# openxrlab/xrsfm

Hardware: AMD Instinct MI355X
Metric: BA iterations/sec x (cams+points) (higher is better)
Workload: dtype f64; 1 GPU; synthetic BAL-style L: 1000 cams / 500000 points / 2000000 obs, GBA accurate (ba_solver.cc:626-629), seed 4; parallelism=single GPU, linear_solver=cholesky (explicit reduced camera matrix, exact)

## Files before the change

xrsfm_amd/csrc/ba_chol.h:

```cpp
#pragma once
#include "ba_kernels.h"
#include "ba_pack.h"

namespace xba {

constexpr int kNB = 64;
constexpr int kLdT = 66;
constexpr int kCamsPerTileDev = 10;

struct CholDev {
    int n, n_pad, T;
    double* S;
    const int* tmap; size_t ld; size_t tstride;
    double* Linv;
    double* y;
    double* rhs;
    double* x;
    const int* cam_off;
    const int* tile_rows;
    int cw, cpt;
};

__device__ __forceinline__ double* tile_ptr(const CholDev& c, int i, int k) {
    return c.tmap ? c.S + (size_t)c.tmap[i * c.T + k] * c.tstride : c.S + (size_t)(i * kNB) * c.ld + k * kNB;
}

typedef double v4d __attribute__((ext_vector_type(4)));

constexpr int kRedLd = 15;

constexpr int kGramTabLd = kGramMaxCams + 1;
static_assert(kTileRunLd == kGramMaxCams, "one run record per distinct camera of a Gram tile (ba_kernels.h: k_gram_runs)");

template <bool UPPER>
__device__ __forceinline__ void pairs_V(const double* F, const double* E, const double* __restrict__ hc, double* V) {
#pragma unroll
    for (int a = 0; a < 6; ++a) {
        const double w0 = F[a] * E[0] + F[6 + a] * E[3], w1 = F[a] * E[1] + F[6 + a] * E[4], w2 = F[a] * E[2] + F[6 + a] * E[5];
        if (UPPER) {
            V[3 * a + 0] = w0 * hc[0];
            V[3 * a + 1] = w0 * hc[1] + w1 * hc[3];
            V[3 * a + 2] = w0 * hc[2] + w1 * hc[4] + w2 * hc[5];
        } else {
            V[3 * a + 0] = w0 * hc[0] + w1 * hc[1] + w2 * hc[2];
            V[3 * a + 1] = w1 * hc[3] + w2 * hc[4];
            V[3 * a + 2] = w2 * hc[5];
        }
    }
}

template <bool UPPER>
__device__ __forceinline__ void pairs_diag(const double* F, const double* V, const double* __restrict__ hc,
                                           const double* __restrict__ g, double* o28) {
    int idx = 0;
#pragma unroll
    for (int a = 0; a < 6; ++a)
#pragma unroll
        for (int c2 = a; c2 < 6; ++c2)
            o28[idx++] = F[a] * F[c2] + F[6 + a] * F[6 + c2]
                         - (V[3 * a] * V[3 * c2] + V[3 * a + 1] * V[3 * c2 + 1] + V[3 * a + 2] * V[3 * c2 + 2]);
    const double g0 = g[0], g1 = g[1], g2 = g[2];
    const double u0 = UPPER ? hc[0] * g0 : hc[0] * g0 + hc[1] * g1 + hc[2] * g2;
    const double u1 = UPPER ? hc[1] * g0 + hc[3] * g1 : hc[3] * g1 + hc[4] * g2;
    const double u2 = UPPER ? hc[2] * g0 + hc[4] * g1 + hc[5] * g2 : hc[5] * g2;
#pragma unroll
    for (int a = 0; a < 6; ++a) o28[21 + a] = -(V[3 * a] * u0 + V[3 * a + 1] * u1 + V[3 * a + 2] * u2);
    o28[27] = 0.0;
}

struct SGroup { int idx, len; double* base; int wld; double ds0, ds1; int dofs; };
template <int NV, typename V>
__device__ __forceinline__ bool sgroup_finish(SGroup g, V (&v)[NV], double* __restrict__ scat, int lane) {
    constexpr int W = sizeof(V) / sizeof(double);
    if (g.idx > 0) {
#pragma unroll
        for (int i = 0; i < NV * W; ++i) g.base[i * kWave + lane] = reinterpret_cast<const double*>(&v[i / W])[i % W];
        g.base[NV * W * kWave + lane] = g.ds0;
        g.base[(NV * W + 1) * kWave + lane] = g.ds1;
    }
    __syncthreads();
    if (g.idx > 0) return false;
    for (int j = 1; j < g.len; ++j) {
        const double* src = g.base + (size_t)j * g.wld;
#pragma unroll
        for (int i = 0; i < NV; ++i) {
            if constexpr (W == 1) v[i] += src[i * kWave + lane];
            else {
#pragma unroll
                for (int q = 0; q < W; ++q) v[i][q] += src[(i * W + q) * kWave + lane];
            }
        }
        g.ds0 += src[NV * W * kWave + lane];
        g.ds1 += src[(NV * W + 1) * kWave + lane];
    }
    if (g.dofs >= 0) { scat[g.dofs] = g.ds0; scat[g.dofs + 14] = g.ds1; }
    return true;
}

template <int NI, int CW = 6>
__device__ __forceinline__ void gram_tile(double* __restrict__ Vst, int R, int Cp, int C, const int* __restrict__ dtab,
                                          double* __restrict__ scat2, int lane, const double (&V)[3 * CW], bool valid, int t, int cidx,
                                          int T, int Th, int passes, bool dense, SGroup sg = SGroup{0, 1, nullptr, 0, 0.0, 0.0, -1},
                                          double* __restrict__ scat = nullptr) {
    static_assert(NI >= 1 && NI <= 4, "a Gram tile has at most 10 cameras = 60 operand rows (ba_pack.h: kGramMaxCams)");
    const int li = lane & 15, lk = lane >> 4;
    v4d acc[NI * (NI + 1) / 2];
#pragma unroll
    for (int p = 0; p < NI * (NI + 1) / 2; ++p) acc[p] = (v4d){0.0, 0.0, 0.0, 0.0};
    const double* rowp[NI];
#pragma unroll
    for (int I = 0; I < NI; ++I) rowp[I] = Vst + min(16 * I + li, R - 1) * Cp + lk;
    for (int h = 0; h < passes; ++h) {
        const int t0 = h * Th, tn = min(Th, T - t0);
        const int C4 = (3 * tn + 3) & ~3;
        if (dense && passes == 1) {
            const int padc = C4 - 3 * tn;
            for (int e = lane; e < R * padc; e += kWave) {
                const int row = e / padc, cc = 3 * tn + (e - row * padc);
                Vst[row * Cp + cc] = 0.0;
            }
        } else {
            for (int e = lane; e < (R * Cp) / 2; e += kWave) reinterpret_cast<double2*>(Vst)[e] = make_double2(0.0, 0.0);
            if (((R * Cp) & 1) && lane == kWave - 1) Vst[R * Cp - 1] = 0.0;
        }
        if (valid && t >= t0 && t < t0 + tn) {
#pragma unroll
            for (int i = 0; i < CW; ++i)
#pragma unroll
                for (int m = 0; m < 3; ++m) Vst[(CW * cidx + i) * Cp + 3 * (t - t0) + m] = V[3 * i + m];
        }
        __builtin_amdgcn_s_waitcnt(0xc07f);
        __builtin_amdgcn_wave_barrier();
        XBA_STAMP(0, 6);
        for (int k0 = 0; k0 < C4; k0 += 4) {
            double a[NI];
#pragma unroll
            for (int I = 0; I < NI; ++I) a[I] = rowp[I][k0];
            int p = 0;
#pragma unroll
            for (int I = 0; I < NI; ++I)
#pragma unroll
                for (int J = 0; J <= I; ++J) { acc[p] = __builtin_amdgcn_mfma_f64_16x16x4f64(a[I], a[J], acc[p], 0, 0, 0); ++p; }
        }
        __builtin_amdgcn_s_waitcnt(0xc07f);
        __builtin_amdgcn_wave_barrier();
    }
    XBA_STAMP(0, 7);
    if (NI <= 2 && sg.len > 1 && !sgroup_finish(sg, acc, scat, lane)) return;
    (void)C; (void)R;
    int tcol[NI], jcol[NI];
#pragma unroll
    for (int J = 0; J < NI; ++J) { const int col = 16 * J + li; const int ra = col / CW; tcol[J] = ra * kGramTabLd; jcol[J] = col - CW * ra; }
    int p = 0;
#pragma unroll
    for (int I = 0; I < NI; ++I) {
// ... 343 lines not shown
                    __builtin_amdgcn_wave_barrier();
                }
            } else if (cp >= 0) {
                double2* out = reinterpret_cast<double2*>(d.scat + 28 * (size_t)cp);
#pragma unroll
                for (int k = 0; k < 14; ++k) out[k] = make_double2(o28[2 * k], o28[2 * k + 1]);
            }
        }
        XBA_STAMP(0, 5);
        const int C = d.tile_ncam[it.first_tile];
        if (GRAM) {
            const unsigned long long headmask = __ballot(s.head);
            const int T = __popcll(headmask);
            const int nvalid = __popcll(__ballot(s.valid));
            const int t = __popcll(headmask & ((2ull << lane) - 1ull)) - 1;
            const int cidx = s.valid ? cidx_raw : 0;
            int passes = 1;
            (void)gram_lds_need(C, T, &passes);
            const int Th = (T + passes - 1) / passes;
            const int R = 6 * C, Rp = (R + 15) & ~15, Cp = ((3 * Th + 3) & ~3) + kGramPad;
            double* Vst = smem;
            int* dtab = reinterpret_cast<int*>(smem + R * Cp);
            dtab[lane] = dt0;
            if (lane + kWave < kGramTabLd * kGramTabLd) dtab[lane + kWave] = dt1;
            const bool dense = nvalid == T * C;
            (void)Rp;
            unsigned short* sched = reinterpret_cast<unsigned short*>(dtab + kGramTabLd * kGramTabLd);
            if (NIK <= 2 && g4_n > 0 && passes == 1) {
                gram4_sched_store(sched, g4_se, lane, g4_n);
                gram_tile4<6>(Vst, R, Cp, C, dtab, scat2, lane, V, s.valid, t, cidx, T, dense, sched, g4_n, sg, d.scat);
            }
            else if (NIK == 0) {
                if (R > 32) gram_tile<3>(Vst, R, Cp, C, dtab, scat2, lane, V, s.valid, t, cidx, T, Th, passes, dense, sg, d.scat);
                else if (R > 16) gram_tile<2>(Vst, R, Cp, C, dtab, scat2, lane, V, s.valid, t, cidx, T, Th, passes, dense, sg, d.scat);
                else gram_tile<1>(Vst, R, Cp, C, dtab, scat2, lane, V, s.valid, t, cidx, T, Th, passes, dense, sg, d.scat);
            }
            else gram_tile<(NIK > 0 ? NIK : 1)>(Vst, R, Cp, C, dtab, scat2, lane, V, s.valid, t, cidx, T, Th, passes, dense, sg, d.scat);
            XBA_STAMP(0, 8);
            return;
        }
        if (GRAM) return;
        if (pair_v) {
            if (s.valid) {
                double2* out = reinterpret_cast<double2*>(pair_v + 18 * (size_t)s.slot);
#pragma unroll
                for (int k = 0; k < 9; ++k) out[k] = make_double2(V[2 * k], V[2 * k + 1]);
            }
            return;
        }
        if (s.valid) {
            pbase = slot_pair_ptr[s.slot];
            npair = slot_pair_ptr[s.slot + 1] - pbase;
        }
        int maxp = npair;
#pragma unroll
        for (int off = 32; off > 0; off >>= 1) maxp = max(maxp, __shfl_xor(maxp, off, kWave));
        for (int dd = 1; dd <= maxp; ++dd) {
            double Vb[18];
#pragma unroll
            for (int k = 0; k < 18; ++k) Vb[k] = __shfl_down(V[k], dd, kWave);
            if (dd <= npair) {
                double2* out = reinterpret_cast<double2*>(scat2 + 36 * (size_t)pair_dst[pbase + dd - 1]);
#pragma unroll
                for (int rb = 0; rb < 6; ++rb) {
                    double o[6];
#pragma unroll
                    for (int ca = 0; ca < 6; ++ca)
                        o[ca] = Vb[3 * rb] * V[3 * ca] + Vb[3 * rb + 1] * V[3 * ca + 1] + Vb[3 * rb + 2] * V[3 * ca + 2];
                    out[3 * rb + 0] = make_double2(o[0], o[1]);
                    out[3 * rb + 1] = make_double2(o[2], o[3]);
                    out[3 * rb + 2] = make_double2(o[4], o[5]);
                }
            }
        }
        return;
    }
    if (GRAM) return;
    const int s_begin = it.first_tile * kWave, s_end = s_begin + it.n_tiles * kWave;
    for (int sa = s_begin + lane; sa < s_end; sa += kWave) {
        if (d.slot_cam[sa] < 0) continue;
        const int pt = d.slot_pt[sa];
        double hc[6];
        {
            const double* hp = (PREP ? d.Hpp : d.Hc) + 6 * (size_t)pt;
            double hv[6];
            for (int k = 0; k < 6; ++k) hv[k] = hp[k];
            if (PREP) point_factor(hv, radius, hc);
            else for (int k = 0; k < 6; ++k) hc[k] = hv[k];
        }
        double Va[18];
        {
            double Fa[12], Ea[6], o28[28], r0, r1;
            load_FE_rc(d, sa, d.slot_cam[sa], pt, Fa, Ea, r0, r1);
            pairs_V<PREP>(Fa, Ea, hc, Va);
            pairs_diag<PREP>(Fa, Va, hc, d.gp + 3 * (size_t)pt, o28);
            double* out = d.scat + 28 * (size_t)d.slot_campos_s[sa];
            for (int k = 0; k < 28; ++k) out[k] = o28[k];
        }
        if (pair_v) {
            double2* out = reinterpret_cast<double2*>(pair_v + 18 * (size_t)sa);
            for (int k = 0; k < 9; ++k) out[k] = make_double2(Va[2 * k], Va[2 * k + 1]);
            continue;
        }
        const int pbase = slot_pair_ptr[sa];
        const int npair = slot_pair_ptr[sa + 1] - pbase;
        for (int dd = 1; dd <= npair; ++dd) {
            const int sb = sa + dd;
            double Fb[12], Eb[6], Vb[18], r0, r1;
            load_FE_rc(d, sb, d.slot_cam[sb], pt, Fb, Eb, r0, r1);
            pairs_V<PREP>(Fb, Eb, hc, Vb);
            double* out = scat2 + 36 * (size_t)pair_dst[pbase + dd - 1];
            for (int rb = 0; rb < 6; ++rb)
                for (int ca = 0; ca < 6; ++ca)
                    out[6 * rb + ca] = Vb[3 * rb] * Va[3 * ca] + Vb[3 * rb + 1] * Va[3 * ca + 1] + Vb[3 * rb + 2] * Va[3 * ca + 2];
        }
    }
}

struct FillLists { const int* tiles; const int* tptr; const int* tent; const double* Sblk; const int* blk_rc;
                   double radius; };
template <int LD>
__device__ __forceinline__ void compose_tile(const CholDev& c, const Dev& d, const FillLists& f, int q, double* A, double* rl) {
    const int ti = f.tiles[2 * q], tj = f.tiles[2 * q + 1];
    const int t = threadIdx.x;
    const int nrows = c.tile_rows[ti];
    for (int e = t; e < kNB * kNB; e += 256) {
        const int r = e >> 6, col = e & 63;
        A[r * LD + col] = (ti == tj && r == col && r >= nrows) ? 1.0 : 0.0;
    }
    if (rl && t < kNB) rl[t] = 0.0;
    __syncthreads();
    const int q0 = f.tptr[q], q1 = f.tptr[q + 1];
    for (int w = t; w < (q1 - q0) * 36; w += 256) {
        const int ent = f.tent[q0 + w / 36], e = w % 36, r = e / 6, col = e % 6;
        if (ent >= 0) {
            const int orow = c.cam_off[f.blk_rc[2 * ent]], ocol = c.cam_off[f.blk_rc[2 * ent + 1]];
            const double v = -f.Sblk[36 * (size_t)ent + e];
            if (orow > ocol) A[((orow & 63) + r) * LD + (ocol & 63) + col] = v;
            else A[((ocol & 63) + col) * LD + (orow & 63) + r] = v;
        } else {
            const int cam = -ent - 1, o = c.cam_off[cam] & 63;
            const double* S = d.camS + 28 * (size_t)cam;
            if (col >= r) {
                double v = S[6 * r - r * (r - 1) / 2 + (col - r)];
                if (r == col) v += f.radius > 0.0 ? clampd(d.camlin[12 * (size_t)cam + r], kLmDiagMin, kLmDiagMax) / f.radius : d.Dc2[6 * (size_t)cam + r];
                A[(o + col) * LD + o + r] = v;
            }
            if (rl && e < 6) rl[o + e] = d.camlin[12 * (size_t)cam + 6 + e] + S[21 + e];
        }
    }
    __syncthreads();
}

__global__ __launch_bounds__(256) void k_tile_fill(CholDev c, Dev d, const int* __restrict__ tiles, const int* __restrict__ tptr,
                                                   const int* __restrict__ tent, const double* __restrict__ Sblk,
                                                   const int* __restrict__ blk_rc, double radius, const int* __restrict__ list = nullptr) {
    __shared__ double A[kNB * (kNB + 1)];
    __shared__ double rl[kNB];
    const FillLists f{tiles, tptr, tent, Sblk, blk_rc, radius};
    const int q = list ? list[blockIdx.x] : (int)blockIdx.x;
    const int ti = tiles[2 * q], tj = tiles[2 * q + 1];
    const int t = threadIdx.x;
    compose_tile<kNB + 1>(c, d, f, q, A, rl);
    double* base = tile_ptr(c, ti, tj);
    for (int e = t; e < kNB * kNB; e += 256) {
        const int r = e >> 6, col = e & 63;
        base[(size_t)r * c.ld + col] = A[r * (kNB + 1) + col];
    }
    if (ti == tj && t < kNB) c.rhs[ti * kNB + t] = rl[t];
}

__global__ void k_sol_gather(CholDev c, double* __restrict__ out, int n_cams) {
    const int i = blockIdx.x * blockDim.x + threadIdx.x;
    if (i < n_cams * c.cw) out[i] = c.x[c.cam_off[i / c.cw] + i % c.cw];
}

__device__ __forceinline__ double readlane_d(double v, int lane) {
    int lo = __double2loint(v), hi = __double2hiint(v);
    lo = __builtin_amdgcn_readlane(lo, lane);
    hi = __builtin_amdgcn_readlane(hi, lane);
    return __hiloint2double(hi, lo);
}
template <int L>
__device__ __forceinline__ double row_bcast_c(double v) {
    int lo = __double2loint(v), hi = __double2hiint(v);
    lo = __builtin_amdgcn_mov_dpp(lo, 0x150 + L, 0xf, 0xf, true);
    hi = __builtin_amdgcn_mov_dpp(hi, 0x150 + L, 0xf, 0xf, true);
    return __hiloint2double(hi, lo);
}
__device__ __forceinline__ double row_bcast(double v, int l) {
    switch (l) {
        case 0: return row_bcast_c<0>(v); case 1: return row_bcast_c<1>(v); case 2: return row_bcast_c<2>(v); case 3: return row_bcast_c<3>(v);
        case 4: return row_bcast_c<4>(v); case 5: return row_bcast_c<5>(v); case 6: return row_bcast_c<6>(v); case 7: return row_bcast_c<7>(v);
        case 8: return row_bcast_c<8>(v); case 9: return row_bcast_c<9>(v); case 10: return row_bcast_c<10>(v); case 11: return row_bcast_c<11>(v);
        case 12: return row_bcast_c<12>(v); case 13: return row_bcast_c<13>(v); case 14: return row_bcast_c<14>(v); default: return row_bcast_c<15>(v);
    }
}
template <int L>
__device__ __forceinline__ double row_bcast64_c(double v) {
    const long long x = __builtin_bit_cast(long long, v);
    const long long r = __builtin_amdgcn_update_dpp((long long)0, x, 0x150 + L, 0xf, 0xf, true);
    return __builtin_bit_cast(double, r);
}
__device__ __forceinline__ double row_bcast64(double v, int l) {
    switch (l) {
        case 0: return row_bcast64_c<0>(v); case 1: return row_bcast64_c<1>(v); case 2: return row_bcast64_c<2>(v); case 3: return row_bcast64_c<3>(v);
        case 4: return row_bcast64_c<4>(v); case 5: return row_bcast64_c<5>(v); case 6: return row_bcast64_c<6>(v); case 7: return row_bcast64_c<7>(v);
        case 8: return row_bcast64_c<8>(v); case 9: return row_bcast64_c<9>(v); case 10: return row_bcast64_c<10>(v); case 11: return row_bcast64_c<11>(v);
        case 12: return row_bcast64_c<12>(v); case 13: return row_bcast64_c<13>(v); case 14: return row_bcast64_c<14>(v); default: return row_bcast64_c<15>(v);
    }
}
#ifndef XBA_POTRF_PV
#define XBA_POTRF_PV 4
#endif
#ifndef XBA_POTRF_OVL
#define XBA_POTRF_OVL 1
#endif
__device__ __forceinline__ void allgather4(double v, double (&out)[4]) {
    const unsigned lo = (unsigned)__double2loint(v), hi = (unsigned)__double2hiint(v);
    const auto l1 = __builtin_amdgcn_permlane16_swap(lo, lo, false, false);
    const auto h1 = __builtin_amdgcn_permlane16_swap(hi, hi, false, false);
    const auto le = __builtin_amdgcn_permlane32_swap(l1[0], l1[0], false, false);
    const auto he = __builtin_amdgcn_permlane32_swap(h1[0], h1[0], false, false);
    const auto lo2 = __builtin_amdgcn_permlane32_swap(l1[1], l1[1], false, false);
    const auto ho2 = __builtin_amdgcn_permlane32_swap(h1[1], h1[1], false, false);
    out[0] = __hiloint2double((int)he[0], (int)le[0]); out[2] = __hiloint2double((int)he[1], (int)le[1]);
    out[1] = __hiloint2double((int)ho2[0], (int)lo2[0]); out[3] = __hiloint2double((int)ho2[1], (int)lo2[1]);
}
struct Panel4 { double a0, a1, a2, a3, x0, x1, x2, x3; };
template <int JJ>
__device__ __forceinline__ void potrf_panel_step(double& ak, double& xk, double& r, double& piv,
                                                 double* a_next, double* x_next, const int n_next) {
    piv = row_bcast64_c<JJ>(ak);
    r = fast_rcp(piv);
    const double tl = ak * r;
    const double xs = xk * r;
    if (n_next >= 1) { const double bv = row_bcast64_c<(JJ + 1) & 15>(ak); a_next[0] = fma(-tl, bv, a_next[0]); x_next[0] = fma(-bv, xs, x_next[0]); }
    if (n_next >= 2) { const double bv = row_bcast64_c<(JJ + 2) & 15>(ak); a_next[1] = fma(-tl, bv, a_next[1]); x_next[1] = fma(-bv, xs, x_next[1]); }
    if (n_next >= 3) { const double bv = row_bcast64_c<(JJ + 3) & 15>(ak); a_next[2] = fma(-tl, bv, a_next[2]); x_next[2] = fma(-bv, xs, x_next[2]); }
}
template <int P>
__device__ __forceinline__ void potrf_panel4(v4d& aa, v4d& ax, bool m1, bool m2, double& Lc, double& Xc, double& Pv) {
    double pa[4], px[4];
    allgather4(aa[P], pa);
    allgather4(ax[P], px);
    double a0 = pa[0], a1 = pa[1], a2 = pa[2], a3 = pa[3], x0 = px[0], x1 = px[1], x2 = px[2], x3 = px[3];
    double r0, r1, r2, r3, j0, j1, j2, j3;
    {
        double an[3] = {a1, a2, a3}, xn[3] = {x1, x2, x3};
        potrf_panel_step<4 * P + 0>(a0, x0, r0, j0, an, xn, 3);
        a1 = an[0]; a2 = an[1]; a3 = an[2]; x1 = xn[0]; x2 = xn[1]; x3 = xn[2];
    }
    {
        double an[3] = {a2, a3, 0.0}, xn[3] = {x2, x3, 0.0};
        potrf_panel_step<4 * P + 1>(a1, x1, r1, j1, an, xn, 2);
        a2 = an[0]; a3 = an[1]; x2 = xn[0]; x3 = xn[1];
    }
    {
        double an[3] = {a3, 0.0, 0.0}, xn[3] = {x3, 0.0, 0.0};
        potrf_panel_step<4 * P + 2>(a2, x2, r2, j2, an, xn, 1);
        a3 = an[0]; x3 = xn[0];
    }
    {
        double an[3] = {0.0, 0.0, 0.0}, xn[3] = {0.0, 0.0, 0.0};
        potrf_panel_step<4 * P + 3>(a3, x3, r3, j3, an, xn, 0);
    }
    auto sel = [&](double v0, double v1, double v2, double v3) { return m2 ? (m1 ? v3 : v2) : (m1 ? v1 : v0); };
    const double a_op = sel(a0, a1, a2, a3), x_op = sel(x0, x1, x2, x3), r_op = sel(r0, r1, r2, r3);
    if (P < 3) {
        const double na = -a_op;
        aa = __builtin_amdgcn_mfma_f64_16x16x4f64(na, a_op * r_op, aa, 0, 0, 0);
        ax = __builtin_amdgcn_mfma_f64_16x16x4f64(na, x_op * r_op, ax, 0, 0, 0);
    }
    Lc = a_op;
    Xc = x_op;
    Pv = sel(j0, j1, j2, j3);
}
__device__ __forceinline__ void potrf_block16_mfma(double (*A)[kLdT], double (*Li)[kLdT], int b0, int lane) {
    const int li = lane & 15, lk = lane >> 4;
    v4d aa, ax;
#pragma unroll
    for (int g = 0; g < 4; ++g) { aa[g] = A[b0 + li][b0 + lk + 4 * g]; ax[g] = (lk + 4 * g == li) ? 1.0 : 0.0; }
    const bool m1 = (lk & 1) != 0, m2 = (lk & 2) != 0;
    double L0, L1, L2, L3, X0, X1, X2, X3, u0, u1, u2, u3;
    potrf_panel4<0>(aa, ax, m1, m2, L0, X0, u0);
    potrf_panel4<1>(aa, ax, m1, m2, L1, X1, u1);
    potrf_panel4<2>(aa, ax, m1, m2, L2, X2, u2);
    potrf_panel4<3>(aa, ax, m1, m2, L3, X3, u3);
    {
        double y0 = __builtin_amdgcn_rsq(u0), y1 = __builtin_amdgcn_rsq(u1), y2 = __builtin_amdgcn_rsq(u2), y3 = __builtin_amdgcn_rsq(u3);
        const double h0 = 0.5 * u0, h1 = 0.5 * u1, h2 = 0.5 * u2, h3 = 0.5 * u3;
#pragma unroll
        for (int it = 0; it < 2; ++it) {
            const double f0 = fma(-h0 * y0, y0, 1.5), f1 = fma(-h1 * y1, y1, 1.5), f2 = fma(-h2 * y2, y2, 1.5), f3 = fma(-h3 * y3, y3, 1.5);
            y0 = y0 * f0; y1 = y1 * f1; y2 = y2 * f2; y3 = y3 * f3;
        }
        L0 *= y0; X0 *= y0; L1 *= y1; X1 *= y1; L2 *= y2; X2 *= y2; L3 *= y3; X3 *= y3;
    }
    A[b0 + li][b0 + lk] = (lk <= li) ? L0 : 0.0;             Li[b0 + lk][b0 + li] = X0;
    A[b0 + li][b0 + 4 + lk] = (4 + lk <= li) ? L1 : 0.0;     Li[b0 + 4 + lk][b0 + li] = X1;
    A[b0 + li][b0 + 8 + lk] = (8 + lk <= li) ? L2 : 0.0;     Li[b0 + 8 + lk][b0 + li] = X2;
    A[b0 + li][b0 + 12 + lk] = (12 + lk <= li) ? L3 : 0.0;   Li[b0 + 12 + lk][b0 + li] = X3;
}

template <int PV>
__device__ __forceinline__ void potrf_block16(double (*A)[kLdT], double (*Li)[kLdT], int b0, int lane) {
    if constexpr (PV == 4) { potrf_block16_mfma(A, Li, b0, lane); return; }
    const int li = lane & 15;
    double a[16];
#pragma unroll
    for (int cc = 0; cc < 16; ++cc) a[cc] = A[b0 + li][b0 + cc];
    double lcol[16];
#pragma unroll
    for (int r = 0; r < 16; ++r) lcol[r] = (r == li) ? 1.0 : 0.0;
#define XBA_POTRF_UPD(cc)                                                \
    {                                                                    \
        const double bv_ = (PV == 1) ? row_bcast64(a[jj], (cc)) : row_bcast(a[jj], (cc));        \
        a[(cc)] = fma(-tl, bv_, a[(cc)]);                                \
        lcol[(cc)] = fma(-bv_, xs, lcol[(cc)]);                          \
        asm volatile("" : "+v"(lcol[(cc)]));    \
    }
    double piv[16];
// ... 439 lines not shown
                                                        double* __restrict__ Wp) {
    __shared__ __attribute__((aligned(16))) double Rs[2][2][kNB * kLdQ];
    __shared__ __attribute__((aligned(16))) double Cs[2][2][kNB * kLdQ];
    __shared__ double yv[2][kNB];
    const int t = threadIdx.x, lane = t & 63, wave = t >> 6, wa = wave >> 1, wb = wave & 1;
    const int o = t >> 2, part = t & 3, li = lane & 15, lk = lane >> 4;
  {
    const int* e = mc + 8 * wg[blockIdx.x];
    const int i0 = e[0], i1 = e[1], k0 = e[2], k1 = e[3], q0 = e[4], q1 = e[5], out0 = e[6], stride = e[7];
    const int ia = wa ? i1 : i0, kb = wb ? k1 : k0;
    const bool active = ia >= 0 && ia >= kb;
    const bool diag = (i0 == k0);
    v4d acc[4][4];
#pragma unroll
    for (int m = 0; m < 4; ++m)
#pragma unroll
        for (int n2 = 0; n2 < 4; ++n2) acc[m][n2] = (v4d){0.0, 0.0, 0.0, 0.0};
    const int i1r = i1 >= 0 ? i1 : i0;
    auto load_step = [&](int st, v2d (&g0)[2], v2d (&g1)[2], v2d (&g2)[2], v2d (&g3)[2]) {
        const int j = q0 + (st >> 2), col = (st & 3) * 16;
        load_quarter_regs(g0, tile_ptr(c, i0, j) + col, c.ld); load_quarter_regs(g1, tile_ptr(c, i1r, j) + col, c.ld);
        load_quarter_regs(g2, tile_ptr(c, k0, j) + col, c.ld); load_quarter_regs(g3, tile_ptr(c, k1, j) + col, c.ld);
    };
    const int ns = 4 * (q1 - q0);
    v2d rg0[2], rg1[2], rg2[2], rg3[2];
    double yreg = 0.0;
    {
        load_step(0, rg0, rg1, rg2, rg3);
        if (diag && t < kNB) yreg = c.y[q0 * kNB + t];
        store_quarter_lds(Rs[0][0], rg0); store_quarter_lds(Rs[0][1], rg1);
        store_quarter_lds(Cs[0][0], rg2); store_quarter_lds(Cs[0][1], rg3);
        if (diag && t < kNB) yv[0][t] = yreg;
        if (ns > 1) {
            load_step(1, rg0, rg1, rg2, rg3);
        }
        __syncthreads();
    }
    double sv0 = 0.0, sv1 = 0.0;
    for (int s = 0; s < ns; ++s) {
        const int buf = s & 1;
        if (s + 1 < ns) {
            store_quarter_lds(Rs[buf ^ 1][0], rg0); store_quarter_lds(Rs[buf ^ 1][1], rg1);
            store_quarter_lds(Cs[buf ^ 1][0], rg2); store_quarter_lds(Cs[buf ^ 1][1], rg3);
            if (diag && ((s + 1) & 3) == 0 && t < kNB) yv[((s + 1) >> 2) & 1][t] = yreg;
        }
        if (s + 2 < ns) {
            load_step(s + 2, rg0, rg1, rg2, rg3);
            if (diag && ((s + 2) & 3) == 0 && t < kNB) yreg = c.y[(q0 + ((s + 2) >> 2)) * kNB + t];
        }
        if (diag) {
            const double* yq = yv[(s >> 2) & 1] + (s & 3) * 16 + part * 4;
#pragma unroll
            for (int m = 0; m < 4; ++m) {
                sv0 += Rs[buf][0][o * kLdQ + part * 4 + m] * yq[m];
                sv1 += Rs[buf][1][o * kLdQ + part * 4 + m] * yq[m];
            }
        }
        if (active) {
            const double* As = Rs[buf][wa];
            const double* Bs = Cs[buf][wb];
#pragma unroll
            for (int kk = 0; kk < 16; kk += 4) {
                double a[4], b[4];
#pragma unroll
                for (int m = 0; m < 4; ++m) {
                    a[m] = As[(16 * m + li) * kLdQ + kk + lk];
                    b[m] = Bs[(16 * m + li) * kLdQ + kk + lk];
                }
#pragma unroll
                for (int m = 0; m < 4; ++m)
#pragma unroll
                    for (int n2 = 0; n2 < 4; ++n2) acc[m][n2] = __builtin_amdgcn_mfma_f64_16x16x4f64(a[m], b[n2], acc[m][n2], 0, 0, 0);
            }
        }
        __syncthreads();
    }
    if (active) {
        double* out = Wp + (size_t)(out0 + (2 * wa + wb) * stride) * kPartStride;
#pragma unroll
        for (int m = 0; m < 4; ++m)
#pragma unroll
            for (int n2 = 0; n2 < 4; ++n2)
#pragma unroll
                for (int g = 0; g < 4; ++g) out[(16 * m + lk + 4 * g) * kNB + 16 * n2 + li] = acc[m][n2][g];
    }
    if (diag) {
        sv0 += __shfl_xor(sv0, 1, kWave); sv0 += __shfl_xor(sv0, 2, kWave);
        sv1 += __shfl_xor(sv1, 1, kWave); sv1 += __shfl_xor(sv1, 2, kWave);
        if (part == 0) {
            Wp[(size_t)out0 * kPartStride + kNB * kNB + o] = sv0;
            if (i1 >= 0) Wp[(size_t)(out0 + 3 * stride) * kPartStride + kNB * kNB + o] = sv1;
        }
    }
  }
}

__device__ __forceinline__ double sum_strided(const double* __restrict__ base, size_t stride, int n) {
    double s = 0.0;
    int p = 0;
    for (; p + 8 <= n; p += 8) {
        double v[8];
#pragma unroll
        for (int u = 0; u < 8; ++u) v[u] = base[(size_t)(p + u) * stride];
        s += ((v[0] + v[1]) + (v[2] + v[3])) + ((v[4] + v[5]) + (v[6] + v[7]));
    }
    for (; p < n; ++p) s += base[(size_t)p * stride];
    return s;
}

template <int EPT>
__device__ __forceinline__ void ll_update_reduce_body(const CholDev& c, const int bx, const int by, const int* __restrict__ rt,
                                                      const int* __restrict__ rp, const double* __restrict__ Wp) {
    const int i = rt[2 * bx], k = rt[2 * bx + 1];
    const int p0 = rp[2 * bx], p1 = rp[2 * bx + 1];
    if (EPT == 1) {
        const int e = by * 256 + threadIdx.x;
        const double s = sum_strided(Wp + (size_t)p0 * kPartStride + e, kPartStride, p1 - p0);
        tile_ptr(c, i, k)[(size_t)(e >> 6) * c.ld + (e & 63)] -= s;
    } else {
        double s[EPT], a0[EPT];
        const double* W = Wp + (size_t)p0 * kPartStride + (size_t)by * EPT * 256 + threadIdx.x;
        double* const tik = tile_ptr(c, i, k);
#pragma unroll
        for (int u = 0; u < EPT; ++u) { s[u] = 0.0; a0[u] = tik[(size_t)(((by * EPT + u) * 256 + threadIdx.x) >> 6) * c.ld + (threadIdx.x & 63)]; }
        int p = p0;
        for (; p + 2 <= p1; p += 2) {
            double v0[EPT], v1[EPT];
#pragma unroll
            for (int u = 0; u < EPT; ++u) { v0[u] = W[(size_t)u * 256]; v1[u] = W[kPartStride + (size_t)u * 256]; }
#pragma unroll
            for (int u = 0; u < EPT; ++u) { s[u] += v0[u]; s[u] += v1[u]; }
            W += 2 * kPartStride;
        }
        if (p < p1) {
#pragma unroll
            for (int u = 0; u < EPT; ++u) s[u] += W[(size_t)u * 256];
        }
#pragma unroll
        for (int u = 0; u < EPT; ++u) {
            const int e = (by * EPT + u) * 256 + threadIdx.x;
            tik[(size_t)(e >> 6) * c.ld + (e & 63)] = a0[u] - s[u];
        }
    }
    if (i == k && by == 0 && threadIdx.x < kNB) {
        const double s = sum_strided(Wp + (size_t)p0 * kPartStride + kNB * kNB + threadIdx.x, kPartStride, p1 - p0);
        c.rhs[k * kNB + threadIdx.x] -= s;
    }
}
__global__ __launch_bounds__(256) void k_ll_update_reduce(CholDev c, const int* __restrict__ rt, const int* __restrict__ rp,
                                                          const double* __restrict__ Wp) {
    ll_update_reduce_body<1>(c, blockIdx.x, blockIdx.y, rt, rp, Wp);
}

struct LvFill { Dev d; FillLists f; const int* fz_q; const int* rest; int n_factor; };
template <bool FILL>
__device__ __forceinline__ void lv_factor_body(const CholDev& c, const int b, const int* __restrict__ tiles, const int* __restrict__ dptr,
                                               const int* __restrict__ dj, const int* __restrict__ tile_cam, double* __restrict__ px,
                                               const LvFill& lf, double (*A)[kLdT], double (*Li)[kLdT], double (*Xs)[kLdT], double (*Tb)[16][17],
                                               double* yv, double* fv, const int* __restrict__ late = nullptr, const double* __restrict__ Ql = nullptr) {
    if (FILL && b >= lf.n_factor) {
        const int q = lf.rest[b - lf.n_factor];
        const int ti = lf.f.tiles[2 * q], tj = lf.f.tiles[2 * q + 1];
        compose_tile<kLdT>(c, lf.d, lf.f, q, &A[0][0], yv);
        double* base = tile_ptr(c, ti, tj);
        for (int e = threadIdx.x; e < kNB * kNB; e += 256) {
            const int r = e >> 6, col = e & 63;
            base[(size_t)r * c.ld + col] = A[r][col];
        }
        if (ti == tj && threadIdx.x < kNB) c.rhs[ti * kNB + threadIdx.x] = yv[threadIdx.x];
        return;
    }
    const int i = tiles[2 * b], k = tiles[2 * b + 1];
    const bool diag = (i == k);
    XBA_STAMP(1, 0);
    const int nb = (c.tile_rows[k] + 15) >> 4;
    const int t = threadIdx.x, lane = t & 63, wave = t >> 6;
    const int li = lane & 15, lk = lane >> 4;
    const int r0 = (wave >> 1) * 32, c0 = (wave & 1) * 32;
    const int o = t >> 2, part = t & 3;
    const size_t ld = c.ld;
    const double* Skk = tile_ptr(c, k, k);
    double* Sik = tile_ptr(c, i, k);
    v4d skk[2][2], sik[2][2], akk[2][2], aik[2][2];
    if (FILL) {
        if (!diag) compose_tile<kLdT>(c, lf.d, lf.f, lf.fz_q[2 * b + 1], &Li[0][0], nullptr);
#pragma unroll
        for (int m = 0; m < 2; ++m)
#pragma unroll
            for (int n2 = 0; n2 < 2; ++n2)
#pragma unroll
                for (int g = 0; g < 4; ++g) {
                    sik[m][n2][g] = diag ? 0.0 : Li[r0 + 16 * m + lk + 4 * g][c0 + 16 * n2 + li];
                    skk[m][n2][g] = 0.0; akk[m][n2][g] = 0.0; aik[m][n2][g] = 0.0;
                }
        __syncthreads();
        compose_tile<kLdT>(c, lf.d, lf.f, lf.fz_q[2 * b], &A[0][0], yv);
    } else {
#pragma unroll
    for (int m = 0; m < 2; ++m)
#pragma unroll
        for (int n2 = 0; n2 < 2; ++n2)
#pragma unroll
            for (int g = 0; g < 4; ++g) {
                const int r = r0 + 16 * m + lk + 4 * g, col = c0 + 16 * n2 + li;
                skk[m][n2][g] = Skk[(size_t)r * ld + col];
                sik[m][n2][g] = diag ? 0.0 : Sik[(size_t)r * ld + col];
                akk[m][n2][g] = 0.0; aik[m][n2][g] = 0.0;
            }
    }
    const int late_kk = (!FILL && late) ? late[2 * b] : -1, late_ik = (!FILL && late) ? late[2 * b + 1] : -1;
    if (late_kk >= 0) {
        const double* Q = Ql + (size_t)late_kk * kPartStride;
#pragma unroll
        for (int m = 0; m < 2; ++m)
#pragma unroll
            for (int n2 = 0; n2 < 2; ++n2)
#pragma unroll
                for (int g = 0; g < 4; ++g) akk[m][n2][g] = Q[(r0 + 16 * m + lk + 4 * g) * kNB + c0 + 16 * n2 + li];
    }
    if (late_ik >= 0) {
        const double* Q = Ql + (size_t)late_ik * kPartStride;
#pragma unroll
        for (int m = 0; m < 2; ++m)
#pragma unroll
            for (int n2 = 0; n2 < 2; ++n2)
#pragma unroll
                for (int g = 0; g < 4; ++g) aik[m][n2][g] = Q[(r0 + 16 * m + lk + 4 * g) * kNB + c0 + 16 * n2 + li];
    }
    double fsum = 0.0;
    if (t < kNB) fv[t] = (diag && late_kk >= 0) ? Ql[(size_t)late_kk * kPartStride + kNB * kNB + t] : 0.0;
    if (!FILL) {
        double* As = &A[0][0]; double* Bs = &Li[0][0];
        const int qa = dptr[b], qb = dptr[b + 1];
        double2 ra[8], rb[8];
        if (qa < qb) {
            const int jj = dj[qa]; const bool own = jj >= 0; const int j = own ? jj : ~jj;
            load_tile_regs(rb, tile_ptr(c, k, j), ld);
            if (!diag && own) load_tile_regs(ra, tile_ptr(c, i, j), ld);
        }
        for (int q = qa; q < qb; ++q) {
            const int jj = dj[q]; const bool own = jj >= 0; const int j = own ? jj : ~jj;
            __syncthreads();
            store_tile_lds(Bs, rb);
            if (!diag && own) store_tile_lds(As, ra);
            if (diag && t < kNB) yv[t] = c.y[j * kNB + t];
            __syncthreads();
            if (q + 1 < qb) {
                const int jn = dj[q + 1]; const bool ownn = jn >= 0; const int j2 = ownn ? jn : ~jn;
                load_tile_regs(rb, tile_ptr(c, k, j2), ld);
                if (!diag && ownn) load_tile_regs(ra, tile_ptr(c, i, j2), ld);
            }
            if (diag) {
#pragma unroll
                for (int m = 0; m < 16; ++m) fsum += Bs[o * kLdT + part * 16 + m] * yv[part * 16 + m];
            }
            tile_abt_mfma(Bs, Bs, akk);
            if (!diag && own) tile_abt_mfma(As, Bs, aik);
        }
        __syncthreads();
        if (diag) {
            fsum += __shfl_xor(fsum, 1, kWave);
            fsum += __shfl_xor(fsum, 2, kWave);
            if (part == 0) fv[o] += fsum;
        }
    }
    XBA_STAMP(1, 1);
    double rhs_k = 0.0;
    if (FILL && t < kNB) rhs_k = yv[t];
#pragma unroll
    for (int m = 0; m < 2; ++m)
#pragma unroll
        for (int n2 = 0; n2 < 2; ++n2)
#pragma unroll
            for (int g = 0; g < 4; ++g) {
                const int r = r0 + 16 * m + lk + 4 * g, col = c0 + 16 * n2 + li;
                if (!FILL) A[r][col] = (col <= r) ? skk[m][n2][g] - akk[m][n2][g] : 0.0;
                Li[r][col] = (r == col && r >= 16 * nb) ? 1.0 : 0.0;
                if (!diag) Xs[r][col] = sik[m][n2][g] - aik[m][n2][g];
            }
    __syncthreads();
    XBA_STAMP(1, 2);
    potrf_lds(A, Li, Tb, nb);
    XBA_STAMP(1, 12);
    if (diag) {
        double* lo = c.Linv + (size_t)k * kNB * kNB;
#pragma unroll
        for (int it = 0; it < 8; ++it) {
            const int e = t + 256 * it; const int r = e >> 5, col = (e & 31) * 2;
            reinterpret_cast<double2*>(lo)[e] = make_double2((col <= r) ? Li[r][col] : 0.0, (col + 1 <= r) ? Li[r][col + 1] : 0.0);
        }
        if (t < kNB) yv[t] = (FILL ? rhs_k : c.rhs[k * kNB + t]) - fv[t];
        __syncthreads();
        double sacc = 0.0;
#pragma unroll
        for (int m = 0; m < 16; ++m) sacc += Li[o][part * 16 + m] * yv[part * 16 + m];
        sacc += __shfl_xor(sacc, 1, kWave);
        sacc += __shfl_xor(sacc, 2, kWave);
        if (part == 0) c.y[k * kNB + o] = sacc;
        if (px) {
            __syncthreads();
            if (part == 0) yv[o] = sacc;
            __syncthreads();
            double s2 = 0.0;
#pragma unroll
            for (int m = 0; m < 16; ++m) s2 += Li[part * 16 + m][o] * yv[part * 16 + m];
            s2 += __shfl_xor(s2, 1, kWave);
            s2 += __shfl_xor(s2, 2, kWave);
            if (part == 0) {
                c.x[k * kNB + o] = s2;
                const int cam = (o < c.cw * c.cpt) ? tile_cam[k * c.cpt + o / c.cw] : -1;
                if (cam >= 0) px[c.cw * (size_t)cam + o % c.cw] = s2;
            }
        }
        XBA_STAMP(1, 13);
        return;
    }
    v4d acc[2][2];
#pragma unroll
    for (int m = 0; m < 2; ++m)
#pragma unroll
        for (int n2 = 0; n2 < 2; ++n2) acc[m][n2] = (v4d){0.0, 0.0, 0.0, 0.0};
    tile_abt_mfma(&Xs[0][0], &Li[0][0], acc);
#pragma unroll
    for (int m = 0; m < 2; ++m)
#pragma unroll
        for (int n2 = 0; n2 < 2; ++n2)
#pragma unroll
            for (int g = 0; g < 4; ++g) Sik[(size_t)(r0 + 16 * m + lk + 4 * g) * ld + c0 + 16 * n2 + li] = acc[m][n2][g];
}
template <bool FILL>
__global__ __launch_bounds__(256) void k_lv_factor(CholDev c, const int* __restrict__ tiles, const int* __restrict__ dptr,
                                                   const int* __restrict__ dj, const int* __restrict__ tile_cam, double* __restrict__ px,
                                                   LvFill lf) {
    __shared__ double A[kNB][kLdT];
    __shared__ double Li[kNB][kLdT];
    __shared__ double Xs[kNB][kLdT];
    __shared__ double Tb[3][16][17];
    __shared__ double yv[kNB], fv[kNB];
    lv_factor_body<FILL>(c, blockIdx.x, tiles, dptr, dj, tile_cam, px, lf, A, Li, Xs, Tb, yv, fv);
}

struct SlotArgs {
    const int* fz_tile; const int* fz_dptr; const int* fz_late; const double* Ql; int n_factor;
    const int* sp_rt; const int* sp_rp; int n_reduce; const double* Wr;
    const int* md_tgt; const int* md_q; int n_late; double* Wq;
    const int* sp_tgt; const int* sp_q; int n_part; double* Wp;
};
__global__ __launch_bounds__(256) void k_panel_slot(CholDev c, SlotArgs a, const int* __restrict__ dj, const int* __restrict__ cj,
                                                    const int* __restrict__ mcj, const int* __restrict__ tile_cam) {
    __shared__ __attribute__((aligned(16))) double T3[3][kNB][kLdT];
    __shared__ double Tb[3][16][17];
    __shared__ double yv[2 * kNB], fv[kNB];
    static_assert(4 * kNB * kLdH <= 3 * kNB * kLdT, "the chunk operands fit the factor tiles");
    const int b = blockIdx.x;
    if (b < a.n_factor) {
        lv_factor_body<false>(c, b, a.fz_tile, a.fz_dptr, dj, tile_cam, nullptr, LvFill{}, T3[0], T3[1], T3[2], Tb, yv, fv, a.fz_late, a.Ql);
    } else if (b < a.n_factor + a.n_late) {
        ll_update_part_body(c, b - a.n_factor, a.md_tgt, a.md_q, mcj, a.Wq, &T3[0][0][0], yv);
    } else if (b < a.n_factor + a.n_late + a.n_part) {
        ll_update_part_body(c, b - a.n_factor - a.n_late, a.sp_tgt, a.sp_q, cj, a.Wp, &T3[0][0][0], yv);
    } else {
        ll_update_reduce_body<16>(c, b - a.n_factor - a.n_late - a.n_part, 0, a.sp_rt, a.sp_rp, a.Wr);
    }
}

__global__ __launch_bounds__(256) void k_lv_bwd(CholDev c, const int* __restrict__ klist, const int* __restrict__ cptr,
                                                const int* __restrict__ ci, const int* __restrict__ tile_cam, double* __restrict__ px) {
    __shared__ double acc[kNB];
    __shared__ int ids[64];
    const int k = klist[blockIdx.x];
    const int t = threadIdx.x, o = t >> 2, part = t & 3;
    const int q0 = cptr[blockIdx.x], q1 = cptr[blockIdx.x + 1];
    const double* Lk = c.Linv + (size_t)k * kNB * kNB;
    double lk[16];
#pragma unroll
    for (int m = 0; m < 16; ++m) lk[m] = Lk[(part * 16 + m) * kNB + o];
    const double yk = c.y[k * kNB + o];
    double s = 0.0;
    for (int qe = q1; qe > q0; qe -= 64) {
        const int qb = max(q0, qe - 64), n = qe - qb;
        __syncthreads();
        if (t < n) ids[t] = ci[qb + t];
        __syncthreads();
#pragma unroll 4
        for (int e = n - 1; e >= 0; --e) {
            const int i = ids[e];
            const double* M = tile_ptr(c, i, k) + (size_t)(part * 16) * c.ld + o;
            const double* xv = c.x + i * kNB + part * 16;
#pragma unroll
            for (int m = 0; m < 16; ++m) s += M[(size_t)m * c.ld] * xv[m];
        }
    }
    s += __shfl_xor(s, 1, kWave);
    s += __shfl_xor(s, 2, kWave);
    if (part == 0) acc[o] = yk - s;
    __syncthreads();
    double s2 = 0.0;
#pragma unroll
    for (int m = 0; m < 16; ++m) s2 += lk[m] * acc[part * 16 + m];
    s2 += __shfl_xor(s2, 1, kWave);
    s2 += __shfl_xor(s2, 2, kWave);
    if (part == 0) {
        c.x[k * kNB + o] = s2;
        const int cam = (o < c.cw * c.cpt) ? tile_cam[k * c.cpt + o / c.cw] : -1;
        if (cam >= 0) px[c.cw * (size_t)cam + o % c.cw] = s2;
    }
}

constexpr int kBwdChunk = 4;
__global__ __launch_bounds__(256) void k_lv_bwd_chunk(CholDev c, const int* __restrict__ klist, const int* __restrict__ ci, const int* __restrict__ tile_cam,
                                                      double* __restrict__ px, const int4* __restrict__ chunks, double* part_buf, unsigned* counter) {
    __shared__ double acc[kNB];
    __shared__ bool last;
    const int4 ch = chunks[blockIdx.x];
    const int k = klist[ch.x], q0 = ch.y, q1 = ch.z, idx = ch.w & 0xffff, nch = ch.w >> 16;
    const int t = threadIdx.x, o = t >> 2, part = t & 3;
    const double* Lk = c.Linv + (size_t)k * kNB * kNB;
    double lk[16];
#pragma unroll
    for (int m = 0; m < 16; ++m) lk[m] = Lk[(part * 16 + m) * kNB + o];
    const double yk = (t < kNB) ? c.y[k * kNB + t] : 0.0;
    double s = 0.0;
    for (int qb = q0; qb < q1; qb += 4) {
        const int n = min(4, q1 - qb);
        double M[4][16], xv[4][16];
#pragma unroll
        for (int u = 0; u < 4; ++u)
            if (u < n) {
                const int i = ci[qb + u];
                const double* Mp = tile_ptr(c, i, k) + (size_t)(part * 16) * c.ld + o;
                const double* xp = c.x + i * kNB + part * 16;
#pragma unroll
                for (int m = 0; m < 16; ++m) { M[u][m] = Mp[(size_t)m * c.ld]; xv[u][m] = xp[m]; }
            }
#pragma unroll
        for (int u = 0; u < 4; ++u)
            if (u < n) {
#pragma unroll
                for (int m = 0; m < 16; ++m) s += M[u][m] * xv[u][m];
            }
    }
    s += __shfl_xor(s, 1, kWave);
    s += __shfl_xor(s, 2, kWave);
    if (nch > 1) {
        double* mine = part_buf + (size_t)blockIdx.x * kNB;
        if (part == 0) __hip_atomic_store(mine + o, s, __ATOMIC_RELAXED, __HIP_MEMORY_SCOPE_AGENT);
        asm volatile("s_waitcnt vmcnt(0)" ::: "memory");
        __syncthreads();
        if (t == 0) last = (__hip_atomic_fetch_add(counter + k, 1u, __ATOMIC_RELAXED, __HIP_MEMORY_SCOPE_AGENT) + 1u == (unsigned)nch);
        __syncthreads();
        if (!last) return;
        __builtin_amdgcn_fence(__ATOMIC_ACQUIRE, "agent");
        if (t < kNB) {
            const double* first = part_buf + (size_t)(blockIdx.x - idx) * kNB + t;
            double sum = 0.0;
            for (int j = 0; j < nch; ++j) sum += __hip_atomic_load(first + (size_t)j * kNB, __ATOMIC_RELAXED, __HIP_MEMORY_SCOPE_AGENT);
            acc[t] = yk - sum;
        }
        if (t == 0) __hip_atomic_store(counter + k, 0u, __ATOMIC_RELAXED, __HIP_MEMORY_SCOPE_AGENT);
    } else {
        if (part == 0) acc[o] = c.y[k * kNB + o] - s;
    }
    __syncthreads();
    double s2 = 0.0;
#pragma unroll
    for (int m = 0; m < 16; ++m) s2 += lk[m] * acc[part * 16 + m];
    s2 += __shfl_xor(s2, 1, kWave);
    s2 += __shfl_xor(s2, 2, kWave);
    if (part == 0) {
        c.x[k * kNB + o] = s2;
        const int cam = (o < c.cw * c.cpt) ? tile_cam[k * c.cpt + o / c.cw] : -1;
        if (cam >= 0) px[c.cw * (size_t)cam + o % c.cw] = s2;
    }
}

typedef __attribute__((address_space(1))) unsigned long long xba_gu64;
constexpr int kBwdPre = 4;
constexpr unsigned kBwdSpinMax = 1u << 21;
__global__ __launch_bounds__(256) void k_lv_bwd_all(CholDev c, const int* __restrict__ klist, const int* __restrict__ cptr, const int* __restrict__ ci,
                                                    const int* __restrict__ tile_cam, double* __restrict__ px, const int* __restrict__ order,
                                                    const unsigned char* __restrict__ col_final, unsigned long long* gx, unsigned* counter,
                                                    unsigned base, unsigned epoch, unsigned* err, double* err_scal, unsigned spin_max,
                                                    unsigned wait_epoch) {
    __shared__ double xs[kBwdPre][kNB];
    __shared__ double acc[kNB];
    __shared__ int s_b;
    const int t = threadIdx.x, o = t >> 2, part = t & 3, lane = t & 63, wave = t >> 6;
    if (t == 0) s_b = (int)(atomicAdd(counter, 1u) - base);
    __syncthreads();
    const int e = order[s_b];
    const int k = klist[e];
    const int q0 = cptr[e], q1 = cptr[e + 1];
    const double* Lk = c.Linv + (size_t)k * kNB * kNB;
    double lk[16];
#pragma unroll
    for (int m = 0; m < 16; ++m) lk[m] = Lk[(part * 16 + m) * kNB + o];
    const double yk = c.y[k * kNB + o];
    double s = 0.0;
    for (int qe = q1; qe > q0; qe -= kBwdPre) {
        const int qb = max(q0, qe - kBwdPre), n = qe - qb;
        double M[kBwdPre][16];
#pragma unroll
        for (int u = 0; u < kBwdPre; ++u)
            if (u < n) {
                const double* Mp = tile_ptr(c, ci[qb + u], k) + (size_t)(part * 16) * c.ld + o;
#pragma unroll
                for (int m = 0; m < 16; ++m) M[u][m] = Mp[(size_t)m * c.ld];
            }
        if (wave < n) {
            const int i = ci[qb + wave];
            double xv;
            if (col_final[i]) xv = c.x[i * kNB + lane];
            else {
                xba_gu64* g = (xba_gu64*)(gx + (size_t)i * (2 * kNB) + 2 * lane);
                unsigned long long a0 = 0, a1 = 0;
                for (unsigned spins = 0;; ++spins) {
                    a0 = __hip_atomic_load(g, __ATOMIC_RELAXED, __HIP_MEMORY_SCOPE_AGENT);
                    a1 = __hip_atomic_load(g + 1, __ATOMIC_RELAXED, __HIP_MEMORY_SCOPE_AGENT);
                    const bool ok = (unsigned)(a0 >> 32) == wait_epoch && (unsigned)(a1 >> 32) == wait_epoch;
                    if (__all(ok)) break;
                    if (spins >= spin_max) { if (lane == 0) { atomicOr(err, 1u); __hip_atomic_store(err_scal, 1.0, __ATOMIC_RELAXED, __HIP_MEMORY_SCOPE_AGENT); } break; }
                    __builtin_amdgcn_s_sleep(1);
                }
                xv = __hiloint2double((int)(unsigned)a1, (int)(unsigned)a0);
            }
            xs[wave][lane] = xv;
        }
        __syncthreads();
#pragma unroll
        for (int u = kBwdPre - 1; u >= 0; --u)
            if (u < n) {
#pragma unroll
                for (int m = 0; m < 16; ++m) s += M[u][m] * xs[u][part * 16 + m];
            }
        __syncthreads();
    }
    s += __shfl_xor(s, 1, kWave);
    s += __shfl_xor(s, 2, kWave);
    if (part == 0) acc[o] = yk - s;
    __syncthreads();
    double s2 = 0.0;
#pragma unroll
    for (int m = 0; m < 16; ++m) s2 += lk[m] * acc[part * 16 + m];
    s2 += __shfl_xor(s2, 1, kWave);
    s2 += __shfl_xor(s2, 2, kWave);
    if (part == 0) {
        xba_gu64* g = (xba_gu64*)(gx + (size_t)k * (2 * kNB) + 2 * o);
        const unsigned long long tag = (unsigned long long)epoch << 32;
        __hip_atomic_store(g, tag | (unsigned)__double2loint(s2), __ATOMIC_RELAXED, __HIP_MEMORY_SCOPE_AGENT);
        __hip_atomic_store(g + 1, tag | (unsigned)__double2hiint(s2), __ATOMIC_RELAXED, __HIP_MEMORY_SCOPE_AGENT);
        c.x[k * kNB + o] = s2;
        const int cam = (o < c.cw * c.cpt) ? tile_cam[k * c.cpt + o / c.cw] : -1;
        if (cam >= 0) px[c.cw * (size_t)cam + o % c.cw] = s2;
    }
}

__global__ void k_zero_vec(double* p, int n) {
    const int i = blockIdx.x * blockDim.x + threadIdx.x;
    if (i < n) p[i] = 0.0;
}

}
```

xrsfm_amd/csrc/ba_plan.h:

```cpp
#pragma once
#include <algorithm>
#include <cstdint>
#include <cstdlib>
#include <utility>
#include <vector>

#include "ba_pack.h"

namespace xba {

constexpr int kPlanTile = 64;
constexpr int kPlanMaxTiles = 4096;
constexpr int kCamsPerTile = 10;
constexpr int kCamsPerTileWide = 7;

struct CholPlan {
    int n = 0, n_pad = 0, T = 0, n_blocks = 0, n_pairs = 0, n_writes = 0, n_tiles_nz = 0, n_levels = 0;
    int n_pair_writes = 0;
    int cam_width = 6, cams_per_tile = kCamsPerTile;
    int ordering = 0;
    long long tile_products = 0;
    int n_hubs = 0, band = 0;
    bool use_levels = false, panel_ll = false;
    bool lookahead = false;
    size_t pairs_shm = 0, pairs_shm_big = 0;
    std::vector<int> pairs_items;
    int n_pairs_small = 0, n_pairs_big = 0, n_pairs_other = 0;
    int gram_n[8] = {0};
    size_t gram_shm[8] = {0};
    std::vector<int> spp, pair_dst, blk_ptr, blk_rc, cam_off, tile_rows, tiles_nz;
    std::vector<int> cols_flat, cols_off;
    std::vector<int> bw2_ent, bw2_off, bw2_link;
    std::vector<int> lv_k, lv_tgt, lv_cptr, lv_cj, lv_bptr, lv_bi;
    std::vector<int> lv_k_off, lv_tgt_off;
    std::vector<int> sp_tgt, sp_q;
    std::vector<int> sp_rt, sp_rp;
    std::vector<int> sp_chunk_off, sp_rt_off;
    int sp_max_chunks = 0;
    int la_depth = 0;
    std::vector<int> sp_slot;
    std::vector<int> sp_e_cnt;
    std::vector<int> mp_chunk, mp_wg, mp_off;
    std::vector<int> tf_ptr, tf_ent;
    std::vector<int> fz_tile, fz_dptr, fz_dj, fz_off;
    std::vector<int> tile_map;
    std::vector<int> md_tgt, md_q, md_cj, md_off, fz_late;
    int md_max = 0;
    std::vector<int> fz_q;
    std::vector<int> fill_rest;
    std::vector<int> tile_cam;
};

struct PairKey {
    unsigned long long first; int second;
    bool operator<(const PairKey& o) const { return first != o.first ? first < o.first : second < o.second; }
};
typedef RawVec<PairKey> PairKeys;

constexpr int kErrDuplicateObs = -100;
constexpr int kErrPlanCheck = -101;

inline int chol_local_keys(const Packed& k, std::vector<int>& spp, PairKeys& keyed) {
    const int ns = k.n_slots;
    const std::vector<long long> cut = pack_cuts(ns, 400000, 64);
    const int nch = (int)cut.size() - 1;
    spp.resize((size_t)ns + 1);
    spp[0] = 0;
    std::vector<long long> total(nch, 0), nkeys(nch, 0);
    pack_parallel_chunks(cut, [&](int t, long long s0, long long s1) {
        int run = 0;
        if (s1 < ns && k.slot_cam[s1] >= 0)
            for (long long s = s1 + 1; s < ns && k.slot_cam[s] >= 0 && k.slot_pt[s] == k.slot_pt[s1]; ++s) ++run;
        long long sum = 0, keys = 0;
        for (long long s = s1 - 1; s >= s0; --s) {
            if (k.slot_cam[s] < 0) run = 0;
            else run = (s + 1 < ns && k.slot_cam[s + 1] >= 0 && k.slot_pt[s + 1] == k.slot_pt[s]) ? run + 1 : 0;
            spp[s + 1] = run;
            sum += run;
            if (k.tile_ncam[s / 64] <= 0) keys += run;
        }
        total[t] = sum; nkeys[t] = keys;
    });
    std::vector<long long> base(nch + 1, 0), kbase(nch + 1, 0);
    for (int t = 0; t < nch; ++t) { base[t + 1] = base[t] + total[t]; kbase[t + 1] = kbase[t] + nkeys[t]; }
    if (base[nch] > INT32_MAX) return XRSFM_BA_EINVAL;
    const int n_obs_pairs = (int)base[nch];
    const std::vector<long long> tcut = pack_cuts(k.n_tiles, 8000, 1);
    const int ntc = (int)tcut.size() - 1;
    std::vector<long long> gkeys(ntc, 0);
    pack_parallel_chunks(tcut, [&](int t, long long t0, long long t1) {
        long long n = 0;
        for (long long tile = t0; tile < t1; ++tile) {
            const int C = k.tile_ncam[tile];
            if (C <= 0) continue;
            const unsigned char* cell = k.gt_cell.data() + k.tile_gt_off[tile];
            for (int a = 0; a < C; ++a)
                for (int b = a + 1; b < C; ++b) n += cell[a * C + b] != 0;
        }
        gkeys[t] = n;
    });
    std::vector<long long> gbase(ntc + 1, kbase[nch]);
    for (int t = 0; t < ntc; ++t) gbase[t + 1] = gbase[t] + gkeys[t];
    if (gbase[ntc] > INT32_MAX) return XRSFM_BA_EINVAL;
    keyed.clear();
    keyed.resize((size_t)gbase[ntc]);
    std::vector<char> bad(nch, 0);
    pack_parallel_chunks(cut, [&](int t, long long s0, long long s1) {
        int acc = (int)base[t];
        PairKey* out = keyed.data() + kbase[t];
        for (long long s = s0; s < s1; ++s) {
            const int start = acc, np = spp[s + 1];
            acc += np;
            spp[s + 1] = acc;
            if (np == 0) continue;
            const bool gram = k.tile_ncam[s / 64] > 0;
            const unsigned long long ca = (unsigned)k.slot_cam[s];
            for (int dd = 1; dd <= np; ++dd) {
                const unsigned long long cb = (unsigned)k.slot_cam[s + dd];
                if (cb <= ca) { bad[t] = 1; return; }
                if (!gram) *out++ = PairKey{(cb << 32) | ca, start + dd - 1};
            }
        }
    });
    for (int t = 0; t < nch; ++t) if (bad[t]) return kErrDuplicateObs;
    pack_parallel_chunks(tcut, [&](int t, long long t0, long long t1) {
        int cams[64];
        PairKey* out = keyed.data() + gbase[t];
        for (long long tile = t0; tile < t1; ++tile) {
            const int C = k.tile_ncam[tile];
            if (C <= 0) continue;
            for (int q = 0; q < 64 && k.slot_cam[64 * tile + q] >= 0; ++q) cams[k.slot_cidx[64 * tile + q]] = k.slot_cam[64 * tile + q];
            const unsigned char* cell = k.gt_cell.data() + k.tile_gt_off[tile];
            for (int a = 0; a < C; ++a)
                for (int b = a + 1; b < C; ++b)
                    if (cell[a * C + b])
                        *out++ = PairKey{((unsigned long long)(unsigned)cams[b] << 32) | (unsigned)cams[a], n_obs_pairs + k.tile_gt_off[tile] + a * C + b};
        }
    });
    if (keyed.size() < 50000) { std::sort(keyed.begin(), keyed.end()); return 0; }
    int cam_bits = 1;
    while (cam_bits < 32 && (1ll << cam_bits) < (long long)k.n_cams) ++cam_bits;
    PairKeys tmp(keyed.size());
    const unsigned hw = std::thread::hardware_concurrency();
    const int nt = (keyed.size() < 2000000 || hw < 2) ? 1 : (int)std::min<unsigned>(16u, hw);
    std::vector<long long> rc(nt + 1);
    for (int t = 0; t <= nt; ++t) rc[t] = (long long)(keyed.size() * (size_t)t / (size_t)nt);
    std::vector<std::vector<unsigned>> hist(nt);
    auto pass = [&](int shift, int bits) {
        const size_t nb = (size_t)1 << bits;
        const unsigned long long mask = nb - 1;
        pack_parallel_chunks(rc, [&](int t, long long i0, long long i1) {
            std::vector<unsigned>& h = hist[t];
            h.assign(nb, 0u);
            for (long long i = i0; i < i1; ++i) h[(keyed[i].first >> shift) & mask]++;
        });
        unsigned run = 0;
        for (size_t b = 0; b < nb; ++b)
            for (int t = 0; t < nt; ++t) { const unsigned v = hist[t][b]; hist[t][b] = run; run += v; }
        pack_parallel_chunks(rc, [&](int t, long long i0, long long i1) {
            std::vector<unsigned>& h = hist[t];
            for (long long i = i0; i < i1; ++i) { const auto& e = keyed[i]; tmp[h[(e.first >> shift) & mask]++] = e; }
        });
        keyed.swap(tmp);
    };
    for (int field = 0; field < 2; ++field)
        for (int done = 0; done < cam_bits; done += 16) pass(32 * field + done, std::min(16, cam_bits - done));
    return 0;
}

namespace plan_detail {
struct CamGraph {
    std::vector<int> ptr, adj;
    int degree(int c) const { return ptr[c + 1] - ptr[c]; }
};
inline CamGraph cam_graph(int Nc, const std::vector<int>& blk_rc, int n_blocks) {
    CamGraph G;
    G.ptr.assign(Nc + 1, 0);
    for (int b = 0; b < n_blocks; ++b) { G.ptr[blk_rc[2 * b] + 1]++; G.ptr[blk_rc[2 * b + 1] + 1]++; }
    for (int c = 0; c < Nc; ++c) G.ptr[c + 1] += G.ptr[c];
    G.adj.resize(G.ptr[Nc]);
    std::vector<int> raw(G.ptr[Nc]), fill(G.ptr.begin(), G.ptr.end() - 1);
    for (int b = 0; b < n_blocks; ++b) {
        const int r = blk_rc[2 * b], c = blk_rc[2 * b + 1];
        raw[fill[r]++] = c; raw[fill[c]++] = r;
    }
    std::vector<int> by_degree(Nc);
    for (int c = 0; c < Nc; ++c) by_degree[c] = c;
    std::sort(by_degree.begin(), by_degree.end(), [&](int a, int b) { return G.degree(a) != G.degree(b) ? G.degree(a) < G.degree(b) : a < b; });
    fill.assign(G.ptr.begin(), G.ptr.end() - 1);
    for (int v : by_degree)
        for (int q = G.ptr[v]; q < G.ptr[v + 1]; ++q) G.adj[fill[raw[q]]++] = v;
    return G;
}
inline std::vector<int> rcm_order(const CamGraph& G) {
    const int Nc = (int)G.ptr.size() - 1;
    const std::vector<int>& ptr = G.ptr;
    const std::vector<int>& adj = G.adj;
    auto degree = [&](int c) { return ptr[c + 1] - ptr[c]; };
    std::vector<int> order; order.reserve(Nc);
    std::vector<int> lvl(Nc, -1), queue;
    std::vector<char> done(Nc, 0);
    auto bfs = [&](int root, int* depth) {
        queue.clear(); queue.push_back(root); lvl[root] = 0;
        size_t head = 0;
// ... 853 lines not shown
```

xrsfm_amd/csrc/xrsfm_ba.hip:

```cpp
#include <dlfcn.h>
#include <hip/hip_runtime.h>

#include <algorithm>
#include <chrono>
#include <condition_variable>
#include <deque>
#include <cmath>
#include <cstdio>
#include <cstdlib>
#include <cstring>
#include <map>
#include <mutex>
#include <thread>
#include <type_traits>
#include <vector>

#include "../../include/xrsfm_ba.h"
#include "ba_chol.h"
#include "ba_cov.h"
#include "ba_filter.h"
#include "ba_kernels.h"
#include "ba_lba.h"
#include "ba_pack.h"
#include "ba_plan.h"
#include "ba_pnp.h"
#include "ba_init.h"
#include "ba_fund.h"
#include "ba_match.h"
#include "ba_refine.h"
#include "ba_tri.h"
#include "ba_trust_region.h"
#include "ba_wide.h"
#include "ba_pack_dev.h"
#include "pose_graph.h"
#include "tag_refine.h"

using namespace xba;
static_assert(kCamsPerTileDev == kCamsPerTile, "k_lv_factor / k_lv_bwd index tile_cam with the device constant, the plan fills it with the host constant");
static_assert(kNB == kPlanTile, "tile size of the kernels (ba_chol.h) and of the plan (ba_plan.h)");

#define HIPCHK(expr)                                                                           \
    do {                                                                                       \
        hipError_t e_ = (expr);                                                                \
        if (e_ != hipSuccess) {                                                                \
            fprintf(stderr, "[xrsfm_ba] HIP error %s at %s:%d: %s\n", hipGetErrorName(e_),   \
                    __FILE__, __LINE__, #expr);                                                \
            return XRSFM_BA_ENODEV;                                                            \
        }                                                                                      \
    } while (0)

namespace {
struct UniqueId { char internal[128]; };
struct Rccl {
    void* lib = nullptr;
    int (*GetUniqueId)(UniqueId*) = nullptr;
    int (*CommInitRank)(void**, int, UniqueId, int) = nullptr;
    int (*AllReduce)(const void*, void*, size_t, int, int, void*, hipStream_t) = nullptr;
    int (*CommDestroy)(void*) = nullptr;
    int (*CommAbort)(void*) = nullptr;
};
Rccl g_rccl;
bool load_rccl() {
    if (g_rccl.lib) return true;
    const char* names[] = {"librccl.so.1", "librccl.so", "/opt/rocm/lib/librccl.so.1"};
    for (const char* n : names) {
        g_rccl.lib = dlopen(n, RTLD_NOW | RTLD_GLOBAL);
        if (g_rccl.lib) break;
    }
    if (!g_rccl.lib) return false;
    g_rccl.GetUniqueId = (int (*)(UniqueId*))dlsym(g_rccl.lib, "ncclGetUniqueId");
    g_rccl.CommInitRank = (int (*)(void**, int, UniqueId, int))dlsym(g_rccl.lib, "ncclCommInitRank");
    g_rccl.AllReduce = (int (*)(const void*, void*, size_t, int, int, void*, hipStream_t))dlsym(g_rccl.lib, "ncclAllReduce");
    g_rccl.CommDestroy = (int (*)(void*))dlsym(g_rccl.lib, "ncclCommDestroy");
    g_rccl.CommAbort = (int (*)(void*))dlsym(g_rccl.lib, "ncclCommAbort");
    return g_rccl.GetUniqueId && g_rccl.CommInitRank && g_rccl.AllReduce && g_rccl.CommDestroy;
}
constexpr int kNcclFloat64 = 8;
constexpr int kNcclSum = 0, kNcclMax = 2;

enum Kid {
    K_LINEARIZE = 0, K_COST, K_CAM_SEGSUM, K_SCHUR_PREP, K_SCHUR_MATVEC, K_PCG_VEC, K_BACKSUB, K_SCHUR_PAIRS, K_BLOCK_SEGSUM,
    K_DENSE_FILL, K_POTRF, K_TRSM, K_UPDATE, K_TRISOLVE, K_LBA, K_SMALL, K_COUNT
};
const char* kKidName[K_COUNT] = {
    "k_linearize", "k_cost", "k_cam_segsum", "k_schur_prep", "k_schur_matvec", "k_pcg_update", "k_backsub", "k_schur_pairs",
    "k_block_segsum", "k_dense_fill", "k_potrf", "k_trsm", "k_update", "k_fwd_bwd", "k_lba_resident", "small_kernels"};

constexpr int kMaxRanks = 64;
constexpr int kCholMaxN = 12288;
constexpr size_t kCholMaxBytes = (size_t)96 << 30;
}

struct CholHost {
    bool ready = false;
    CholDev dev{};
    int n_blocks = 0, n_pairs = 0, n_tiles_nz = 0, T = 0;
    int *slot_pair_ptr = nullptr, *pair_dst = nullptr, *blk_ptr = nullptr, *blk_rc = nullptr;
    double *scat2 = nullptr, *Sblk = nullptr;
    bool bwd_push = false;
    bool bwd_chunk = false; int4* bc_chunks = nullptr; std::vector<int> bc_off; double* bc_part = nullptr; unsigned* bc_ctr = nullptr;
    int gram4 = 1;
    bool pair_from_v = false; int2* ent_src = nullptr; double* pair_v = nullptr;
    int* tiles_nz = nullptr;
    size_t pairs_shm = 0, pairs_shm_big = 0;
    int* pairs_items = nullptr; int n_pairs_small = 0, n_pairs_big = 0, n_pairs_other = 0;
    int gram_n[8] = {0}; size_t gram_shm[8] = {0};
    bool gram_merge = true;
    int sgroup = 1; int* sgrp = nullptr;
    hipStream_t aux = nullptr; hipEvent_t ev_fork = nullptr, ev_join = nullptr;
    int* cols_flat = nullptr;
    std::vector<int> cols_off;
    int* bw2_ent = nullptr; std::vector<int> bw2_off, bw2_link;
    bool use_levels = false, panel_ll = false;
    bool lookahead = false;
    int n_levels = 0;
    int *lv_k = nullptr, *lv_tgt = nullptr, *lv_cptr = nullptr, *lv_cj = nullptr;
    int *lv_bptr = nullptr, *lv_bi = nullptr;
    std::vector<int> lv_k_off, lv_tgt_off;
    int* bw_order = nullptr; unsigned char* bw_final = nullptr; unsigned long long* bw_gx = nullptr; unsigned* bw_ctr = nullptr;
    bool bw_debug_timeout = false;
    int bw_n = 0; unsigned bw_launches = 0; bool bwd_all = false;
    int *sp_tgt = nullptr, *sp_q = nullptr, *sp_rt = nullptr, *sp_rp = nullptr;
    int* sp_slot = nullptr;
    int la_depth = 0; std::vector<int> sp_e_cnt; std::vector<hipEvent_t> la_ev_factor, la_ev_early;
    std::vector<int> sp_chunk_off, sp_rt_off, mp_off;
    int *mp_chunk = nullptr, *mp_wg = nullptr;
    double* sp_work = nullptr; int sp_max_chunks = 0;
    int *fz_tile = nullptr, *fz_dptr = nullptr, *fz_dj = nullptr, *tile_cam = nullptr;
    int *md_tgt = nullptr, *md_q = nullptr, *md_cj = nullptr, *fz_late = nullptr;
    std::vector<int> md_off; int md_max = 0; double* md_work = nullptr;
    int *fz_q = nullptr, *fill_rest = nullptr; int n_fill_rest = 0;
    bool rest_apart = false;
    int32_t facts[16] = {0};
    bool S_filled = false;
    std::vector<int> fz_off;
    int *tf_ptr = nullptr, *tf_ent = nullptr;
    std::vector<int> cam_off_host;
    std::vector<int> tile_map_host; size_t S_doubles = 0;
    std::vector<int> lv_k_host, lv_bptr_host, lv_bi_host;
    int ordering = 0;
};

struct xrsfm_ba_context {
    int device = 0;
    hipStream_t stream = nullptr;
    Packed pk;
    Dev d{};
    std::vector<void*> allocs;
    std::vector<size_t> alloc_class;
    CamRec* cam0 = nullptr; double* P0 = nullptr;
    int n_points_caller = 0;
    double* h_scal = nullptr;
    double* h_scal_dev = nullptr;
    unsigned long long seq = 0;
    PcgStatus* h_st = nullptr;
    void* comm = nullptr; int n_ranks = 1, rank = 0;
    xrsfm_ba_allreduce_fn hook = nullptr; void* hook_user = nullptr; std::vector<double> hook_buf;
    bool multi() const { return comm != nullptr || hook != nullptr; }
    bool profiling = false;
    std::vector<hipEvent_t> ev_pool; size_t ev_used = 0;
    struct Rec { int kid; size_t e0; int tag; };
    std::vector<Rec> recs;
    double prof_ms[K_COUNT] = {0}; int prof_n[K_COUNT] = {0};
    bool dev_packed = false; int host_pack_level = 2;
    int* dpk_slot_obs = nullptr; unsigned char* dpk_gt_cell = nullptr;
    bool linearized = false;
    unsigned long long debug_stall_ticks = 0;
    bool poisoned = false;
    bool fused = true;
    bool wide = false;
    DevW w{};
    std::vector<int> cam_intr_host;
    bool pcg_coarse = true; double* pcg_w = nullptr;
    bool prep_fused = true;
    double step_radius = 0.0;
    bool step_prep = false;
    bool backsub_lean = true;
    int* long_items = nullptr; int n_long = 0;
    bool step_valid = false;
    bool backsub_done = false;
    bool gradmax_done = false, published = false;
    double* part2 = nullptr; unsigned* ticket = nullptr;
    struct LinBuf { double* rt = nullptr; double* Jp = nullptr; CamLin* camrec = nullptr; double* Hpp = nullptr; double* gp = nullptr; double* camlin = nullptr; } alt;
    double* jbuf[4] = {nullptr, nullptr, nullptr, nullptr};
    std::vector<unsigned long long> pattern_keys;
    bool have_pattern = false;
    CholHost chol;
};

namespace {

struct DevCache {
    std::mutex mu;
    std::map<std::pair<int, size_t>, std::vector<void*>> free_blocks;
    size_t cached_bytes = 0;
    static size_t size_class(size_t bytes) {
        size_t c = 256;
        while (c < bytes) c += (c < (1u << 20)) ? c : c / 4;
        return c;
    }
    void* get(int dev, size_t bytes, size_t* cls) {
        *cls = size_class(bytes);
        {
            std::lock_guard<std::mutex> g(mu);
            auto it = free_blocks.find({dev, *cls});
            if (it != free_blocks.end() && !it->second.empty()) { void* p = it->second.back(); it->second.pop_back(); cached_bytes -= *cls; return p; }
        }
        void* p = nullptr;
        if (hipMalloc(&p, *cls) != hipSuccess) {
            release_all();
            if (hipMalloc(&p, *cls) != hipSuccess) return nullptr;
        }
        return p;
    }
    void put(int dev, void* p, size_t cls) {
        std::lock_guard<std::mutex> g(mu);
        if (cached_bytes + cls > (size_t)16 << 30) { (void)hipFree(p); return; }
        free_blocks[{dev, cls}].push_back(p); cached_bytes += cls;
    }
    void release_all() {
        std::lock_guard<std::mutex> g(mu);
        for (auto& kv : free_blocks) for (void* p : kv.second) (void)hipFree(p);
        free_blocks.clear(); cached_bytes = 0;
    }
};
DevCache g_cache;

struct HostBundle { hipStream_t stream; double* h_scal; PcgStatus* h_st; hipStream_t aux = nullptr; hipEvent_t ev_fork = nullptr, ev_join = nullptr; };
static void bundle_release(const HostBundle& b) {
    (void)hipHostFree(b.h_scal); (void)hipHostFree(b.h_st); (void)hipStreamDestroy(b.stream);
    if (b.aux) { (void)hipStreamDestroy(b.aux); (void)hipEventDestroy(b.ev_fork); (void)hipEventDestroy(b.ev_join); }
}
struct BundleCache {
    std::mutex mu;
    std::map<int, std::vector<HostBundle>> free_bundles;
    bool get(int dev, HostBundle* b) {
        {
            std::lock_guard<std::mutex> g(mu);
            auto& v = free_bundles[dev];
            if (!v.empty()) { *b = v.back(); v.pop_back(); return true; }
        }
        *b = HostBundle{nullptr, nullptr, nullptr};
        if (hipStreamCreate(&b->stream) != hipSuccess) return false;
        if (hipHostMalloc((void**)&b->h_scal, sizeof(double) * (S_COUNT + 2), hipHostMallocMapped | hipHostMallocCoherent) != hipSuccess ||
            hipHostMalloc((void**)&b->h_st, sizeof(PcgStatus)) != hipSuccess) {
            if (b->h_scal) (void)hipHostFree(b->h_scal);
            (void)hipStreamDestroy(b->stream);
            return false;
        }
        return true;
    }
    void put(int dev, const HostBundle& b) {
        std::lock_guard<std::mutex> g(mu);
        auto& v = free_bundles[dev];
        if (v.size() >= 8) { bundle_release(b); return; }
        v.push_back(b);
    }
};
BundleCache g_bundles;

struct PinnedPool {
    std::mutex mu;
    std::vector<std::pair<void*, size_t>> free_blocks;
    void* get(size_t bytes, size_t* cap) {
        {
            std::lock_guard<std::mutex> g(mu);
            size_t best = free_blocks.size();
            for (size_t i = 0; i < free_blocks.size(); ++i)
                if (free_blocks[i].second >= bytes && (best == free_blocks.size() || free_blocks[i].second < free_blocks[best].second)) best = i;
            if (best < free_blocks.size()) { void* p = free_blocks[best].first; *cap = free_blocks[best].second; free_blocks.erase(free_blocks.begin() + best); return p; }
        }
        size_t c = 1 << 16;
        while (c < bytes) c *= 2;
        void* p = nullptr;
        if (hipHostMalloc(&p, c, hipHostMallocDefault) != hipSuccess) return nullptr;
        *cap = c;
        return p;
    }
    void put(void* p, size_t cap) {
        std::lock_guard<std::mutex> g(mu);
        if (free_blocks.size() >= 8 || cap > ((size_t)256 << 20)) { (void)hipHostFree(p); return; }
        free_blocks.push_back({p, cap});
    }
    void release_all() {
        std::lock_guard<std::mutex> g(mu);
        for (auto& b : free_blocks) (void)hipHostFree(b.first);
        free_blocks.clear();
    }
};
// ... 443 lines not shown
    unsigned char* drop = nullptr;
    int *flag = nullptr, *pos = nullptr, *cflag = nullptr, *cpos = nullptr, *campos_s = nullptr, *camptr_s = nullptr, *blk_tmp = nullptr;
    if ((e = dev_alloc(c, &h.sgrp, (size_t)n_merged)) || (e = dev_alloc(c, &drop, (size_t)std::max(1, nt))) ||
        (e = dev_alloc(c, &flag, (size_t)n_ent + 1)) || (e = dev_alloc(c, &pos, (size_t)n_ent + 1)) ||
        (e = dev_alloc(c, &cflag, (size_t)n_cent + 1)) || (e = dev_alloc(c, &cpos, (size_t)n_cent + 1)) ||
        (e = dev_alloc(c, &campos_s, (size_t)std::max(1, ns))) || (e = dev_alloc(c, &camptr_s, (size_t)Nc + 1)) ||
        (e = dev_alloc(c, &blk_tmp, (size_t)h.n_blocks + 1))) return e;
    hipStream_t st = c->stream;
    HIPCHK(hipMemsetAsync(drop, 0, (size_t)std::max(1, nt), st));
    HIPCHK(hipMemsetAsync(flag, 0, sizeof(int) * ((size_t)n_ent + 1), st));
    HIPCHK(hipMemsetAsync(cflag, 0, sizeof(int) * ((size_t)n_cent + 1), st));
    hipLaunchKernelGGL(k_sgroup_table, dim3(cdiv(n_merged, 256)), dim3(256), 0, st, (const int*)h.pairs_items, n_merged, G, d.tile_stride, d.tile_ncam,
                       d.slot_cam, d.slot_cidx, h.sgrp, drop);
    if (ns > 0) hipLaunchKernelGGL(k_sgroup_cam_flags, dim3(cdiv(ns, 256)), dim3(256), 0, st, d.slot_campos_g, (const unsigned char*)drop, ns, cflag);
    if (n_obs_pairs > 0) hipLaunchKernelGGL(k_sgroup_pair_flags, dim3(cdiv(n_obs_pairs, 256)), dim3(256), 0, st, (const int*)h.pair_dst, n_obs_pairs, flag);
    if (nt > 0) hipLaunchKernelGGL(k_sgroup_cell_flags, dim3(cdiv(nt, 256)), dim3(256), 0, st, (const int*)(h.pair_dst + n_obs_pairs), d.tile_ncam, d.tile_gt_off,
                                   (const unsigned char*)drop, nt, flag);
    HIPCHK(hipGetLastError());
    auto scan = [&](int* in, int* out, size_t n) -> int {
        size_t q = 0;
        if (rocprim::exclusive_scan(nullptr, q, in, out, 0, n, rocprim::plus<int>(), st) != hipSuccess) return XRSFM_BA_ENODEV;
        unsigned char* tmp = nullptr;
        if (int e2 = dev_alloc(c, &tmp, std::max<size_t>(q, 1))) return e2;
        return rocprim::exclusive_scan(tmp, q, in, out, 0, n, rocprim::plus<int>(), st) == hipSuccess ? 0 : XRSFM_BA_ENODEV;
    };
    if ((e = scan(flag, pos, (size_t)n_ent + 1)) || (e = scan(cflag, cpos, (size_t)n_cent + 1))) return e;
    int n_cent_s = n_cent;
    HIPCHK(hipMemcpyAsync(&n_cent_s, cpos + n_cent, sizeof(int), hipMemcpyDeviceToHost, st));
    HIPCHK(hipStreamSynchronize(st));
    if (!ge && 4LL * (n_cent - n_cent_s) < (long long)n_cent) { h.sgroup = 1; h.sgrp = nullptr; return 0; }
    if (ns > 0) hipLaunchKernelGGL(k_sgroup_remap, dim3(cdiv(ns, 256)), dim3(256), 0, st, d.slot_campos_g, ns, (const int*)cflag, (const int*)cpos, campos_s);
    hipLaunchKernelGGL(k_sgroup_remap_ptr, dim3(cdiv(Nc + 1, 256)), dim3(256), 0, st, d.cam_ptr_g, Nc + 1, (const int*)cpos, camptr_s);
    if (h.n_pairs > 0) hipLaunchKernelGGL(k_sgroup_remap, dim3(cdiv(h.n_pairs, 256)), dim3(256), 0, st, (const int*)h.pair_dst, h.n_pairs, (const int*)flag, (const int*)pos, h.pair_dst);
    hipLaunchKernelGGL(k_sgroup_remap_ptr, dim3(cdiv(h.n_blocks + 1, 256)), dim3(256), 0, st, (const int*)h.blk_ptr, h.n_blocks + 1, (const int*)pos, blk_tmp);
    HIPCHK(hipGetLastError());
    HIPCHK(hipMemcpyAsync(h.blk_ptr, blk_tmp, sizeof(int) * ((size_t)h.n_blocks + 1), hipMemcpyDeviceToDevice, st));
    HIPCHK(hipMemcpyAsync(&n_writes, pos + n_ent, sizeof(int), hipMemcpyDeviceToHost, st));
    HIPCHK(hipStreamSynchronize(st));
    d.slot_campos_s = campos_s; d.cam_ptr_s = camptr_s;
    return 0;
}

static bool chol_packed_storage(const CholPlan& P) {
    const char* packed_e = std::getenv("XRSFM_BA_PACKED");
    if (packed_e) return packed_e[0] != '0';
    return (size_t)P.n_pad * P.n_pad * sizeof(double) > ((size_t)4 << 30);
}

struct BwdChoice { bool all, chunk, push; };
static BwdChoice chol_bwd_choice(const CholPlan& P) {
    const char* be = std::getenv("XRSFM_BA_BWD_ALL");
    const char* bce = std::getenv("XRSFM_BA_BWD_CHUNK");
    BwdChoice b{};
    b.all = !(be && be[0] == '0') && P.use_levels && !P.panel_ll && P.n_levels >= 2;
    const bool deep = P.use_levels && !P.panel_ll && !b.all && P.n_levels > 32;
    b.chunk = deep && !(bce && bce[0] == '0');
    b.push = deep && !b.chunk;
    return b;
}

constexpr int kFillRestApart = 4096;
static bool chol_rest_apart(const CholPlan& P) {
    return !P.lookahead && (int)P.fill_rest.size() > kFillRestApart;
}

static void chol_plan_facts(const CholPlan& P, int32_t f[16]) {
    const BwdChoice bw = chol_bwd_choice(P);
    int n_macro = 0, n_split = 0;
    for (int lv = 0; lv < P.n_levels; ++lv) {
        if ((int)P.mp_off.size() > lv + 1 && P.mp_off[lv + 1] - P.mp_off[lv] - 1 > 0) ++n_macro;
        if ((int)P.sp_rt_off.size() > lv + 1 && P.sp_rt_off[lv + 1] > P.sp_rt_off[lv]) ++n_split;
    }
    int bwd;
    if (P.lookahead || ((P.panel_ll || bw.push) && P.T > 1)) bwd = 4;
    else if (P.panel_ll || bw.push) bwd = 0;
    else if (bw.chunk) bwd = 3;
    else if (bw.all) bwd = 2;
    else bwd = P.n_levels >= 2 ? 1 : 0;
    int heights = 0;
    for (int t = 0; t < P.T && t < (int)P.tile_rows.size(); ++t) heights |= 1 << (P.tile_rows[t] / P.cam_width);
    const int32_t v[16] = {P.T, P.n_levels, P.ordering, P.lookahead ? 2 : (P.panel_ll ? 1 : 0), n_macro, n_split, P.la_depth,
                           (int32_t)P.fill_rest.size(), chol_rest_apart(P) ? 1 : 0, chol_packed_storage(P) ? 1 : 0, bwd, heights,
                           P.cam_width, P.n_blocks, P.n, P.n_tiles_nz};
    for (int i = 0; i < 16; ++i) f[i] = v[i];
}

int chol_setup(xrsfm_ba_context* c) {
    CholHost& h = c->chol;
    if (h.ready) return 0;
    const Packed& k = c->pk;
    const int Nc = k.n_cams;
    std::vector<int> spp;
    PairKeys keyed;
    PhaseTimer timer("chol setup");
    int e = 0;
    devpack::KeysResult KR;
    PlanPrebuilt pre;
    bool dev_keys = false;
    {
        const char* dk = std::getenv("XRSFM_BA_DEVICE_KEYS");
        dev_keys = c->dev_packed && !c->wide && c->n_ranks == 1 && !c->have_pattern && !(dk && dk[0] == '0');
    }
    if (dev_keys) {
        std::vector<std::pair<void*, size_t>> scratch;
        auto keep = [&](size_t bytes) -> void* { unsigned char* q = nullptr; return dev_alloc(c, &q, bytes) ? nullptr : (void*)q; };
        auto scr = [&](size_t bytes) -> void* { size_t cls = 0; void* q = g_cache.get(c->device, bytes, &cls); if (q) scratch.push_back({q, cls}); return q; };
        e = devpack::device_keys(k, c->d.slot_cam, c->d.slot_pt, c->d.slot_cidx, c->d.tile_ncam, c->d.tile_gt_off, c->dpk_gt_cell, c->stream, keep, scr, KR);
        (void)hipStreamSynchronize(c->stream);
        for (auto& b : scratch) g_cache.put(c->device, b.first, b.second);
        if (e) return e;
        if (KR.duplicate) return kErrDuplicateObs;
        pre.n_pairs = KR.n_pairs; pre.n_writes = KR.n_writes; pre.n_pair_writes = KR.n_pair_writes; pre.blk_rc = KR.blk_rc_host; pre.n_other = KR.n_other;
        for (int b = 0; b < 8; ++b) { pre.gram_n[b] = KR.gram_n[b]; pre.gram_shm[b] = KR.gram_shm[b]; }
    } else {
        if ((e = ensure_host_pack(c, 1))) return e;
        e = chol_local_keys(k, spp, keyed);
        if (e) return e;
    }
    timer.mark("pair keys");
    if (c->n_ranks > 1 && !c->have_pattern) {
        std::vector<double> occ((size_t)Nc * Nc, 0.0);
        for (const auto& kv : keyed) occ[(size_t)(kv.first >> 32) * Nc + (kv.first & 0xffffffffu)] = 1.0;
        double* d_occ = nullptr;
        if (hipMalloc((void**)&d_occ, occ.size() * sizeof(double)) != hipSuccess) return XRSFM_BA_ENOMEM;
        int e2 = XRSFM_BA_OK;
        if (hipMemcpy(d_occ, occ.data(), occ.size() * sizeof(double), hipMemcpyHostToDevice) != hipSuccess) e2 = XRSFM_BA_ENODEV;
        if (!e2) e2 = allreduce(c, d_occ, occ.size(), kNcclMax);
        if (!e2 && hipStreamSynchronize(c->stream) != hipSuccess) e2 = XRSFM_BA_ENODEV;
        if (!e2 && hipMemcpy(occ.data(), d_occ, occ.size() * sizeof(double), hipMemcpyDeviceToHost) != hipSuccess) e2 = XRSFM_BA_ENODEV;
        (void)hipFree(d_occ);
        if (e2) return e2;
        c->pattern_keys.clear();
        for (int rb = 0; rb < Nc; ++rb)
            for (int ca = 0; ca < rb; ++ca)
                if (occ[(size_t)rb * Nc + ca] > 0.0) c->pattern_keys.push_back(((unsigned long long)rb << 32) | (unsigned)ca);
        c->have_pattern = true;
    }
    CholPlan P;
    try { e = chol_plan_build(k, spp, keyed, c->have_pattern ? &c->pattern_keys : nullptr, P, kCholMaxN, kCholMaxBytes, c->wide ? kW : 6, dev_keys ? &pre : nullptr); }
    catch (const std::bad_alloc&) { return XRSFM_BA_ENOMEM; }
    if (e) return e == kErrPlanCheck ? XRSFM_BA_EINTERNAL : e;
    timer.mark("plan");
    if (P.n > kCholMaxN && !(P.use_levels || P.ordering >= 2)) return XRSFM_BA_ETOOBIG;
    h.n_blocks = P.n_blocks; h.n_pairs = P.n_pairs; h.T = P.T; h.n_tiles_nz = P.n_tiles_nz; h.n_levels = P.n_levels;
    h.use_levels = P.use_levels; h.panel_ll = P.panel_ll; h.lookahead = P.lookahead; h.ordering = P.ordering; h.pairs_shm = P.pairs_shm; h.pairs_shm_big = P.pairs_shm_big; h.n_pairs_small = P.n_pairs_small; h.n_pairs_big = P.n_pairs_big; h.n_pairs_other = P.n_pairs_other; h.cam_off_host = P.cam_off;
    for (int b = 0; b < 8; ++b) { h.gram_n[b] = P.gram_n[b]; h.gram_shm[b] = P.gram_shm[b]; }
    { const char* me = std::getenv("XRSFM_BA_GRAM_MERGE"); h.gram_merge = !(me && me[0] == '0'); }
    h.cols_off = P.cols_off; h.bw2_off = P.bw2_off; h.bw2_link = P.bw2_link;
    h.lv_k_off = P.lv_k_off; h.lv_tgt_off = P.lv_tgt_off;
    h.lv_k_host = P.lv_k; h.lv_bptr_host = P.lv_bptr; h.lv_bi_host = P.lv_bi;
    h.sp_chunk_off = P.sp_chunk_off; h.sp_rt_off = P.sp_rt_off; h.mp_off = P.mp_off; h.fz_off = P.fz_off;
    int *d_cam_off = nullptr, *d_tile_rows = nullptr, *d_tmap = nullptr;
#define TRYC(x) do { e = (x); if (e) return e; } while (0)
    BatchUpload up(c);
    if (dev_keys) { h.slot_pair_ptr = KR.spp; h.pair_dst = KR.pair_dst; h.blk_ptr = KR.blk_ptr; h.blk_rc = KR.blk_rc; }
    else { up.add(&h.slot_pair_ptr, P.spp); up.add(&h.pair_dst, P.pair_dst); up.add(&h.blk_ptr, P.blk_ptr); up.add(&h.blk_rc, P.blk_rc); }
    up.add(&h.tiles_nz, P.tiles_nz); up.add(&h.cols_flat, P.cols_flat); up.add(&h.bw2_ent, P.bw2_ent);
    up.add(&h.lv_k, P.lv_k); up.add(&h.lv_tgt, P.lv_tgt); up.add(&h.lv_cptr, P.lv_cptr);
    up.add(&h.lv_cj, P.lv_cj);
    up.add(&h.lv_bptr, P.lv_bptr); up.add(&h.lv_bi, P.lv_bi);
    up.add(&h.sp_tgt, P.sp_tgt); up.add(&h.sp_q, P.sp_q); up.add(&h.mp_chunk, P.mp_chunk); up.add(&h.mp_wg, P.mp_wg);
    up.add(&h.sp_rt, P.sp_rt); up.add(&h.sp_rp, P.sp_rp); up.add(&h.sp_slot, P.sp_slot);
    h.la_depth = P.la_depth; h.sp_e_cnt = P.sp_e_cnt;
    up.add(&h.tf_ptr, P.tf_ptr); up.add(&h.tf_ent, P.tf_ent);
    up.add(&h.fz_tile, P.fz_tile); up.add(&h.fz_dptr, P.fz_dptr); up.add(&h.fz_dj, P.fz_dj);
    up.add(&h.fz_q, P.fz_q); up.add(&h.fill_rest, P.fill_rest); h.n_fill_rest = (int)P.fill_rest.size();
    up.add(&h.md_tgt, P.md_tgt); up.add(&h.md_q, P.md_q); up.add(&h.md_cj, P.md_cj); up.add(&h.fz_late, P.fz_late);
    h.md_off = P.md_off; h.md_max = P.md_max;
    up.add(&h.tile_cam, P.tile_cam);
    if (dev_keys) h.pairs_items = KR.pairs_items; else up.add(&h.pairs_items, P.pairs_items);
    h.sp_max_chunks = P.sp_max_chunks;
    TRYC(dev_alloc(c, &h.sp_work, (size_t)std::max(1, P.sp_max_chunks) * kPartStride * (P.lookahead ? 2 : (P.la_depth > 0 ? P.la_depth + 1 : 1))));
    if (P.lookahead) TRYC(dev_alloc(c, &h.md_work, (size_t)std::max(1, P.md_max) * kPartStride * 2));
    up.add(&d_cam_off, P.cam_off); up.add(&d_tile_rows, P.tile_rows); up.add(&d_tmap, P.tile_map);
    TRYC(up.flush());
    timer.mark("uploads");
    int n_writes = P.n_writes;
    TRYC(sgroup_setup(c, n_writes));
    const size_t blk_vals = c->wide ? kWB : 36, cam_vals = c->wide ? kWS : 28;
    {
        double* both = nullptr;
        TRYC(dev_alloc(c, &both, (size_t)Nc * cam_vals + (size_t)(P.n_blocks > 0 ? P.n_blocks : 1) * blk_vals));
        if (c->wide) c->w.camS = both; else c->d.camS = both;
        h.Sblk = both + (size_t)Nc * cam_vals;
    }
    {
        const char* g4 = std::getenv("XRSFM_BA_GRAM4");
        h.gram4 = !(g4 && g4[0] == '0');
        const char* pe = std::getenv("XRSFM_BA_PAIR_V");
        h.pair_from_v = !c->wide && h.n_pairs_other > 0 && (pe ? pe[0] != '0' : (P.n_pair_writes >= 262144 && 2LL * P.n_pair_writes >= n_writes));
        const size_t n_scat2 = h.pair_from_v ? (size_t)std::max(0, n_writes - P.n_pair_writes) : (size_t)std::max(0, n_writes);
        TRYC(dev_alloc(c, &h.scat2, std::max<size_t>(1, n_scat2) * blk_vals));
        if (h.pair_from_v) {
            const size_t ne = (size_t)std::max(1, n_writes);
            TRYC(dev_alloc(c, &h.ent_src, ne));
            TRYC(dev_alloc(c, &h.pair_v, (size_t)std::max(1, k.n_slots) * 18));
            HIPCHK(hipMemsetAsync(h.ent_src, 0xff, sizeof(int2) * ne, c->stream));
            hipLaunchKernelGGL(k_pair_sources, dim3(h.n_pairs_other), dim3(kWave), 0, c->stream, c->d, (const int*)(h.pairs_items + h.n_pairs_small + h.n_pairs_big),
                               (const int*)h.slot_pair_ptr, (const int*)h.pair_dst, h.ent_src);
            HIPCHK(hipGetLastError());
            const int n_cells = c->pk.n_gt_cells;
            if (n_cells > 0) {
                const int nb = cdiv(n_cells, 256);
                int* block_off = nullptr;
                TRYC(dev_alloc(c, &block_off, (size_t)nb));
                int* cells = h.pair_dst + (h.n_pairs - n_cells);
                hipLaunchKernelGGL(k_gram_compact_count, dim3(nb), dim3(256), 0, c->stream, (const int*)cells, n_cells, block_off);
                hipLaunchKernelGGL(k_gram_compact_scan, dim3(1), dim3(64), 0, c->stream, block_off, nb);
                hipLaunchKernelGGL(k_gram_compact, dim3(nb), dim3(256), 0, c->stream, cells, n_cells, h.ent_src, (const int*)block_off);
                HIPCHK(hipGetLastError());
            }
        }
    }
    h.dev.n = P.n; h.dev.n_pad = P.n_pad; h.dev.T = P.T; h.dev.cam_off = d_cam_off; h.dev.tile_rows = d_tile_rows;
    h.dev.cw = P.cam_width; h.dev.cpt = P.cams_per_tile;
    const bool packed = chol_packed_storage(P);
    h.rest_apart = chol_rest_apart(P);
    chol_plan_facts(P, h.facts);
    h.dev.tmap = packed ? d_tmap : nullptr;
    h.dev.ld = packed ? (size_t)kNB : (size_t)P.n_pad;
    h.dev.tstride = (size_t)kNB * kNB + kNB;
    h.S_doubles = packed ? ((size_t)P.n_tiles_nz + 1) * h.dev.tstride : (size_t)P.n_pad * P.n_pad;
    if (h.S_doubles * sizeof(double) > kCholMaxBytes) return XRSFM_BA_ETOOBIG;
    h.tile_map_host = P.tile_map;
    TRYC(dev_alloc(c, &h.dev.S, h.S_doubles));
    TRYC(dev_alloc(c, &h.dev.Linv, (size_t)P.T * kNB * kNB));
    TRYC(dev_alloc(c, &h.dev.y, (size_t)P.n_pad)); TRYC(dev_alloc(c, &h.dev.rhs, (size_t)P.n_pad)); TRYC(dev_alloc(c, &h.dev.x, (size_t)P.n_pad));
    {
        const BwdChoice bw = chol_bwd_choice(P);
        h.bwd_all = bw.all; h.bwd_chunk = bw.chunk; h.bwd_push = bw.push;
        { const char* te = std::getenv("XRSFM_BA_DEBUG_BWD_TIMEOUT"); h.bw_debug_timeout = te && te[0] == '1'; }
        if (h.bwd_chunk) {
            std::vector<int4> chunks;
            h.bc_off.assign(P.n_levels + 1, 0);
            int max_lv = 1;
            for (int lv = 0; lv < P.n_levels; ++lv) {
                for (int e2 = P.lv_k_off[lv]; e2 < P.lv_k_off[lv + 1]; ++e2) {
                    const int q0 = P.lv_bptr[e2], q1 = P.lv_bptr[e2 + 1];
                    const int nch = std::max(1, (q1 - q0 + kBwdChunk - 1) / kBwdChunk);
                    for (int j = 0; j < nch; ++j) chunks.push_back(make_int4(e2, q0 + j * kBwdChunk, std::min(q1, q0 + (j + 1) * kBwdChunk), j | (nch << 16)));
                }
                h.bc_off[lv + 1] = (int)chunks.size();
                max_lv = std::max(max_lv, h.bc_off[lv + 1] - h.bc_off[lv]);
            }
            TRYC(dev_upload(c, &h.bc_chunks, chunks));
            TRYC(dev_alloc(c, &h.bc_part, (size_t)max_lv * kNB)); TRYC(dev_alloc(c, &h.bc_ctr, (size_t)P.T));
            HIPCHK(hipMemsetAsync(h.bc_ctr, 0, sizeof(unsigned) * (size_t)P.T, c->stream));
        }
        if (h.bwd_all) {
            std::vector<int> order;
            std::vector<unsigned char> fin(P.T, 0);
            for (int lv = P.n_levels - 2; lv >= 0; --lv)
                for (int e2 = P.lv_k_off[lv]; e2 < P.lv_k_off[lv + 1]; ++e2) order.push_back(e2);
            for (int e2 = P.lv_k_off[P.n_levels - 1]; e2 < P.lv_k_off[P.n_levels]; ++e2) fin[P.lv_k[e2]] = 1;
            h.bw_n = (int)order.size(); h.bw_launches = 0;
            TRYC(dev_upload(c, &h.bw_order, order)); TRYC(dev_upload(c, &h.bw_final, fin));
            TRYC(dev_alloc(c, &h.bw_gx, (size_t)P.T * 2 * kNB)); TRYC(dev_alloc(c, &h.bw_ctr, (size_t)2));
            HIPCHK(hipMemsetAsync(h.bw_gx, 0, sizeof(unsigned long long) * (size_t)P.T * 2 * kNB, c->stream));
            HIPCHK(hipMemsetAsync(h.bw_ctr, 0, sizeof(unsigned) * 2, c->stream));
        }
    }
#undef TRYC
    HIPCHK(hipMemsetAsync(h.dev.S, 0, sizeof(double) * h.S_doubles, c->stream));
    const int shm = 2 * kNB * kLdT * (int)sizeof(double);
    set_kernel_attributes(c->device);
    if ((h.n_pairs_other > 0 || h.la_depth > 0) && !h.aux) {
        if (hipStreamCreateWithFlags(&h.aux, hipStreamNonBlocking) != hipSuccess) h.aux = nullptr;
        if (h.aux && (hipEventCreateWithFlags(&h.ev_fork, hipEventDisableTiming) != hipSuccess ||
                      hipEventCreateWithFlags(&h.ev_join, hipEventDisableTiming) != hipSuccess)) {
            if (h.ev_fork) (void)hipEventDestroy(h.ev_fork);
            (void)hipStreamDestroy(h.aux); h.aux = nullptr; h.ev_fork = h.ev_join = nullptr;
        }
    }
    if (h.la_depth > 0) {
        bool ok = h.aux != nullptr;
        h.la_ev_factor.assign(h.n_levels, nullptr); h.la_ev_early.assign(h.n_levels, nullptr);
        for (int lv = 0; lv < h.n_levels && ok; ++lv)
            ok = hipEventCreateWithFlags(&h.la_ev_factor[lv], hipEventDisableTiming) == hipSuccess &&
                 hipEventCreateWithFlags(&h.la_ev_early[lv], hipEventDisableTiming) == hipSuccess;
        if (!ok) {
            for (hipEvent_t e2 : h.la_ev_factor) if (e2) (void)hipEventDestroy(e2);
            for (hipEvent_t e2 : h.la_ev_early) if (e2) (void)hipEventDestroy(e2);
            h.la_ev_factor.clear(); h.la_ev_early.clear();
        }
    }
    timer.mark("allocations + attributes");
    h.ready = true;
    return 0;
}

int chol_assemble(xrsfm_ba_context* c, bool materialize = false) {
    Dev& d = c->d;
    CholHost& h = c->chol;
    const int n_obs_pairs = h.n_pairs - c->pk.n_gt_cells;
    {
        Timed t_(c, K_SCHUR_PAIRS);
        const bool fork = h.n_pairs_other > 0 && h.aux;
        const double radius = c->step_radius;
        auto launch_other = [&](hipStream_t st) {
            const int* items = h.pairs_items + h.n_pairs_small + h.n_pairs_big;
            double* pv = h.pair_from_v ? h.pair_v : nullptr;
            if (c->step_prep) hipLaunchKernelGGL((k_schur_pairs<false, true, 0>), dim3(h.n_pairs_other), dim3(kWave), h.pairs_shm, st, d, items, h.slot_pair_ptr, h.pair_dst, n_obs_pairs, h.scat2, radius, pv);
            else hipLaunchKernelGGL((k_schur_pairs<false, false, 0>), dim3(h.n_pairs_other), dim3(kWave), h.pairs_shm, st, d, items, h.slot_pair_ptr, h.pair_dst, n_obs_pairs, h.scat2, radius, pv);
        };
        auto launch_gram = [&](auto ni, int n, size_t shm, const int* items, hipStream_t st) {
            constexpr int NI = decltype(ni)::value;
            const int G = NI == 0 ? h.sgroup : 1;
            const size_t wbytes = (shm + 15) & ~(size_t)15;
            const dim3 grid(cdiv(n, G)), block(kWave * G);
            const size_t shm_wg = G > 1 ? wbytes * G : shm;
            const int wld = G > 1 ? (int)(wbytes / sizeof(double)) : 0;
            const int* sg = G > 1 ? (const int*)h.sgrp : nullptr;
            if (c->step_prep) hipLaunchKernelGGL((k_schur_pairs<true, true, NI>), grid, block, shm_wg, st, d, items, h.slot_pair_ptr, h.pair_dst, n_obs_pairs, h.scat2, radius, (double*)nullptr, h.gram4, sg, n, wld);
            else hipLaunchKernelGGL((k_schur_pairs<true, false, NI>), grid, block, shm_wg, st, d, items, h.slot_pair_ptr, h.pair_dst, n_obs_pairs, h.scat2, radius, (double*)nullptr, h.gram4, sg, n, wld);
        };
        int n_merged = 0; size_t shm_merged = 0;
        for (int b = 0; b < 6; ++b) { n_merged += h.gram_n[b]; if (h.gram_n[b] > 0) shm_merged = std::max(shm_merged, h.gram_shm[b]); }
        const bool merge = h.gram_merge && n_merged > 0;
        constexpr bool gram_fork = true;
        int big = -1;
        for (int b = 0; b < 8; ++b) if (h.gram_n[b] > 0 && (big < 0 || h.gram_n[b] > h.gram_n[big])) big = b;
        if (merge) big = -2;
        auto launch_buckets = [&](bool main_side) {
            const int* items = h.pairs_items;
            if (merge && main_side) launch_gram(std::integral_constant<int, 0>{}, n_merged, shm_merged, items, c->stream);
            for (int b = 0; b < 8; ++b) {
                const int n = h.gram_n[b];
                const bool on_main = !(fork && gram_fork) || b == big;
                if (n > 0 && on_main == main_side && !(merge && b < 6)) {
                    hipStream_t st = on_main ? c->stream : h.aux;
                    switch (b >> 1) {
                        case 0: launch_gram(std::integral_constant<int, 1>{}, n, h.gram_shm[b], items, st); break;
                        case 1: launch_gram(std::integral_constant<int, 2>{}, n, h.gram_shm[b], items, st); break;
                        case 2: launch_gram(std::integral_constant<int, 3>{}, n, h.gram_shm[b], items, st); break;
                        default: launch_gram(std::integral_constant<int, 4>{}, n, h.gram_shm[b], items, st); break;
                    }
                }
                items += n;
            }
        };
        if (fork) {
            HIPCHK(hipEventRecord(h.ev_fork, c->stream));
            launch_buckets(true);
            HIPCHK(hipStreamWaitEvent(h.aux, h.ev_fork, 0));
            launch_other(h.aux);
            launch_buckets(false);
            HIPCHK(hipEventRecord(h.ev_join, h.aux));
            HIPCHK(hipStreamWaitEvent(c->stream, h.ev_join, 0));
        } else {
            if (h.n_pairs_other > 0) launch_other(c->stream);
            launch_buckets(true);
        }
    }
    if (d.n_cams + h.n_blocks > 0) {
        if (h.pair_from_v) LAUNCH(c, K_BLOCK_SEGSUM, k_chol_segsum_v, dim3(d.n_cams + (h.n_blocks + 3) / 4), dim3(kBlock), 0, d.scat, d.cam_ptr_s, d.camS, d.n_cams, h.scat2, h.blk_ptr, h.Sblk,
                                  h.n_blocks, (const int2*)h.ent_src, (const double*)h.pair_v);
        else LAUNCH(c, K_BLOCK_SEGSUM, k_chol_segsum, dim3(d.n_cams + h.n_blocks), dim3(kBlock), 0, d.scat, d.cam_ptr_s, d.camS, d.n_cams, h.scat2, h.blk_ptr, h.Sblk);
    }
    int e = allreduce(c, d.camS, (size_t)d.n_cams * 28 + (size_t)h.n_blocks * 36, kNcclSum);
    if (e) return e;
    h.S_filled = materialize;
    if (h.S_filled && h.n_tiles_nz > 0)
        LAUNCH(c, K_DENSE_FILL, k_tile_fill, dim3(h.n_tiles_nz), dim3(256), 0, h.dev, d, h.tiles_nz, h.tf_ptr, h.tf_ent, h.Sblk, h.blk_rc,
               c->step_prep ? c->step_radius : 0.0);
    return 0;
}

static void panel_backward(xrsfm_ba_context* c) {
    CholHost& h = c->chol;
    const int T = h.T;
    int k = T - 1;
    for (int p = 0; k >= 1; k -= 2, ++p) {
            const int n = h.bw2_off[p + 1] - h.bw2_off[p];
            LAUNCH(c, K_TRISOLVE, k_bwd2, dim3(1 + n), dim3(256), 0, h.dev, k, h.bw2_link[p], (const int*)(h.bw2_ent + 2 * (size_t)h.bw2_off[p]));
        }
    for (; k >= 0; --k) {
        const int ncol = h.cols_off[k + 1] - h.cols_off[k];
        LAUNCH(c, K_TRISOLVE, k_bwd, dim3(1 + ncol), dim3(256), 0, h.dev, k, h.cols_flat + h.cols_off[k]);
    }
}

int chol_factor_solve(xrsfm_ba_context* c) {
    Dev& d = c->d;
    CholHost& h = c->chol;
    const int T = h.T;
    double* px_out = c->wide ? c->w.px : d.px;
    const size_t shm = 2 * (size_t)kNB * kLdT * sizeof(double);
    if (h.lookahead) {
        auto chunks = [&](int lv) { return lv < h.n_levels ? h.sp_chunk_off[lv + 1] - h.sp_chunk_off[lv] : 0; };
        auto targets = [&](int lv) { return lv < h.n_levels ? h.sp_rt_off[lv + 1] - h.sp_rt_off[lv] : 0; };
        auto lates = [&](int lv) { return lv < h.n_levels ? h.md_off[lv + 1] - h.md_off[lv] : 0; };
        double* const Wbuf[2] = {h.sp_work, h.sp_work + (size_t)std::max(1, h.sp_max_chunks) * kPartStride};
        double* const Qbuf[2] = {h.md_work, h.md_work + (size_t)std::max(1, h.md_max) * kPartStride};
        for (int s2 = 0; s2 < h.n_levels; ++s2) {
            const int nf = h.fz_off[s2 + 1] - h.fz_off[s2];
            SlotArgs a{};
            const int lr = s2 + 1, lp = s2 + 2;
            a.n_reduce = targets(lr);
            if (a.n_reduce > 0) { a.sp_rt = h.sp_rt + 2 * (size_t)h.sp_rt_off[lr]; a.sp_rp = h.sp_rp + 2 * (size_t)h.sp_rt_off[lr]; a.Wr = Wbuf[lr & 1]; }
            a.n_part = chunks(lp);
            if (a.n_part > 0) { a.sp_tgt = h.sp_tgt + 2 * (size_t)h.sp_chunk_off[lp]; a.sp_q = h.sp_q + 2 * (size_t)h.sp_chunk_off[lp]; a.Wp = Wbuf[lp & 1]; }
            a.n_late = lates(lr);
            if (a.n_late > 0) { a.md_tgt = h.md_tgt + 2 * (size_t)h.md_off[lr]; a.md_q = h.md_q + 2 * (size_t)h.md_off[lr]; a.Wq = Qbuf[lr & 1]; }
            if (s2 == 0 && !h.S_filled) {
                LvFill lf{};
                lf.d = d; lf.f = FillLists{h.tiles_nz, h.tf_ptr, h.tf_ent, h.Sblk, h.blk_rc, c->step_prep ? c->step_radius : 0.0};
                lf.fz_q = h.fz_q; lf.rest = h.fill_rest; lf.n_factor = nf;
                if (nf + h.n_fill_rest > 0)
                    LAUNCH(c, K_POTRF, k_lv_factor<true>, dim3(nf + h.n_fill_rest), dim3(256), 0, h.dev, h.fz_tile, h.fz_dptr, h.fz_dj,
                           (const int*)h.tile_cam, (double*)nullptr, lf);
                if (a.n_reduce + a.n_part + a.n_late > 0) return XRSFM_BA_EINTERNAL;
                continue;
            }
            a.fz_tile = h.fz_tile + 2 * (size_t)h.fz_off[s2]; a.fz_dptr = h.fz_dptr + h.fz_off[s2]; a.n_factor = nf;
            a.fz_late = h.fz_late + 2 * (size_t)h.fz_off[s2]; a.Ql = Qbuf[s2 & 1];
            const int nwg = a.n_factor + a.n_reduce + a.n_late + a.n_part;
            if (nwg > 0) LAUNCH(c, K_POTRF, k_panel_slot, dim3(nwg), dim3(256), 0, h.dev, a, (const int*)h.fz_dj, (const int*)h.lv_cj, (const int*)h.md_cj, (const int*)h.tile_cam);
        }
        panel_backward(c);
        if (d.n_cams > 0) LAUNCH(c, K_SMALL, k_sol_gather, dim3(cdiv((long long)d.n_cams * h.dev.cw, 256)), dim3(256), 0, h.dev, px_out, d.n_cams);
        return 0;
    }
    if (h.use_levels || h.panel_ll) {
        for (int lv = 0; lv < h.n_levels; ++lv) {
            const int nt = h.lv_tgt_off[lv + 1] - h.lv_tgt_off[lv];
            const int nch = h.sp_chunk_off[lv + 1] - h.sp_chunk_off[lv], nmc = h.mp_off[lv + 1] - h.mp_off[lv] - 1;
            const int nrt = h.sp_rt_off[lv + 1] - h.sp_rt_off[lv];
            const bool la_on = h.la_depth > 0 && !h.la_ev_factor.empty();
            const int n_early = la_on ? h.sp_e_cnt[lv] : 0;
            double* const Wlv = h.sp_work + (h.la_depth > 0 ? (size_t)(lv % (h.la_depth + 1)) * (size_t)std::max(1, h.sp_max_chunks) * kPartStride : 0);
            if (nmc > 0)
                LAUNCH(c, K_UPDATE, k_panel2_part, dim3(nmc), dim3(256), 0, h.dev, h.mp_chunk, h.mp_wg + h.mp_off[lv], h.sp_work);
            else if (nch - n_early > 0)
                LAUNCH(c, K_UPDATE, k_ll_update_part, dim3(nch - n_early), dim3(256), 0, h.dev, h.sp_tgt + 2 * (size_t)(h.sp_chunk_off[lv] + n_early),
                       h.sp_q + 2 * (size_t)(h.sp_chunk_off[lv] + n_early), h.lv_cj, Wlv, (const int*)(h.sp_slot + h.sp_chunk_off[lv] + n_early));
            if (n_early > 0) HIPCHK(hipStreamWaitEvent(c->stream, h.la_ev_early[lv], 0));
            if (nrt > 0)
                LAUNCH(c, K_UPDATE, k_ll_update_reduce, dim3(nrt, 16), dim3(256), 0, h.dev, h.sp_rt + 2 * (size_t)h.sp_rt_off[lv],
                       h.sp_rp + 2 * (size_t)h.sp_rt_off[lv], Wlv);
            const int nf = h.fz_off[lv + 1] - h.fz_off[lv];
            const bool with_bwd = ((!h.panel_ll && !h.bwd_push && !h.bwd_chunk) || T == 1) && lv == h.n_levels - 1;
            LvFill lf{};
            if (lv == 0 && !h.S_filled) {
                lf.d = d; lf.f = FillLists{h.tiles_nz, h.tf_ptr, h.tf_ent, h.Sblk, h.blk_rc, c->step_prep ? c->step_radius : 0.0};
                lf.fz_q = h.fz_q; lf.rest = h.fill_rest; lf.n_factor = nf;
                const bool rest_apart = h.rest_apart;
                if (rest_apart)
                    LAUNCH(c, K_DENSE_FILL, k_tile_fill, dim3(h.n_fill_rest), dim3(256), 0, h.dev, d, h.tiles_nz, h.tf_ptr, h.tf_ent, h.Sblk, h.blk_rc,
                           c->step_prep ? c->step_radius : 0.0, (const int*)h.fill_rest);
                const int n_rest = rest_apart ? 0 : h.n_fill_rest;
                if (nf + n_rest > 0)
                    LAUNCH(c, K_POTRF, k_lv_factor<true>, dim3(nf + n_rest), dim3(256), 0, h.dev, h.fz_tile, h.fz_dptr, h.fz_dj,
                           (const int*)h.tile_cam, with_bwd ? px_out : (double*)nullptr, lf);
            } else if (nf > 0)
                LAUNCH(c, K_POTRF, k_lv_factor<false>, dim3(nf), dim3(256), 0, h.dev, h.fz_tile + 2 * (size_t)h.fz_off[lv], h.fz_dptr + h.fz_off[lv], h.fz_dj,
                       (const int*)h.tile_cam, with_bwd ? px_out : (double*)nullptr, lf);
            if (la_on) {
                const int le = lv + 1 + h.la_depth;
                const int ne = le < h.n_levels ? h.sp_e_cnt[le] : 0;
                if (ne > 0) {
                    HIPCHK(hipEventRecord(h.la_ev_factor[lv], c->stream));
                    HIPCHK(hipStreamWaitEvent(h.aux, h.la_ev_factor[lv], 0));
                    double* const Wle = h.sp_work + (size_t)(le % (h.la_depth + 1)) * (size_t)std::max(1, h.sp_max_chunks) * kPartStride;
                    {
                        Timed t_(c, K_UPDATE, -1, h.aux);
                        hipLaunchKernelGGL(k_ll_update_part, dim3(ne), dim3(256), 0, h.aux, h.dev, h.sp_tgt + 2 * (size_t)h.sp_chunk_off[le],
                                           h.sp_q + 2 * (size_t)h.sp_chunk_off[le], h.lv_cj, Wle, (const int*)(h.sp_slot + h.sp_chunk_off[le]));
                    }
                    HIPCHK(hipEventRecord(h.la_ev_early[le], h.aux));
                }
            }
        }
        if (h.panel_ll || h.bwd_push) {
            if (T == 1) return 0;
            panel_backward(c);
            if (d.n_cams > 0) LAUNCH(c, K_SMALL, k_sol_gather, dim3(cdiv((long long)d.n_cams * h.dev.cw, 256)), dim3(256), 0, h.dev, px_out, d.n_cams);
            return 0;
        }
        if (h.bwd_chunk) {
            for (int lv = h.n_levels - 1; lv >= 0; --lv) {
                const int n = h.bc_off[lv + 1] - h.bc_off[lv];
                if (n > 0) LAUNCH(c, K_TRISOLVE, k_lv_bwd_chunk, dim3(n), dim3(256), 0, h.dev, (const int*)h.lv_k, (const int*)h.lv_bi, (const int*)h.tile_cam, px_out,
                                  (const int4*)(h.bc_chunks + h.bc_off[lv]), h.bc_part, h.bc_ctr);
            }
            return 0;
        }
        if (h.bwd_all && h.bw_n > 0) {
            const unsigned base = h.bw_launches * (unsigned)h.bw_n;
            const unsigned epoch = ++h.bw_launches;
            LAUNCH(c, K_TRISOLVE, k_lv_bwd_all, dim3(h.bw_n), dim3(256), 0, h.dev, (const int*)h.lv_k, (const int*)h.lv_bptr, (const int*)h.lv_bi,
                   (const int*)h.tile_cam, px_out, (const int*)h.bw_order, (const unsigned char*)h.bw_final, h.bw_gx, h.bw_ctr, base, epoch, h.bw_ctr + 1,
                   d.scal + S_BWD_ERR, h.bw_debug_timeout ? 64u : kBwdSpinMax, h.bw_debug_timeout ? epoch + 1u : epoch);
            return 0;
        }
        for (int lv = h.n_levels - 2; lv >= 0; --lv) {
            const int nk = h.lv_k_off[lv + 1] - h.lv_k_off[lv];
            LAUNCH(c, K_TRISOLVE, k_lv_bwd, dim3(nk), dim3(256), 0, h.dev, h.lv_k + h.lv_k_off[lv], h.lv_bptr + h.lv_k_off[lv], h.lv_bi, h.tile_cam, px_out);
        }
        return 0;
    }
    return XRSFM_BA_EINTERNAL;
}

Dev candidate_view(const xrsfm_ba_context* c) {
    Dev v = c->d;
    std::swap(v.cam, v.cam_cand); std::swap(v.P, v.P_cand);
    v.rt = c->alt.rt; v.Jp = c->alt.Jp; v.camrec = c->alt.camrec; v.Hpp = c->alt.Hpp; v.gp = c->alt.gp; v.camlin = c->alt.camlin;
    v.part = c->d.part + 4 * (size_t)c->d.n_items;
    return v;
}
void accept_candidate(xrsfm_ba_context* c) {
    Dev& d = c->d;
    std::swap(d.cam, d.cam_cand); std::swap(d.P, d.P_cand);
    std::swap(d.rt, c->alt.rt); std::swap(d.Jp, c->alt.Jp); std::swap(d.camrec, c->alt.camrec);
    std::swap(d.Hpp, c->alt.Hpp); std::swap(d.gp, c->alt.gp); std::swap(d.camlin, c->alt.camlin);
}

void launch_backsub(xrsfm_ba_context* c, int nbi, int nbc, CamLin* cr, bool want_yp) {
    Dev& d = c->d;
    const dim3 grid(nbi + nbc), block(kBlock);
    if (!c->backsub_lean) {
        if (c->step_prep) LAUNCH(c, K_BACKSUB, k_backsub_parent<true>, grid, block, 0, d, nbi, cr, c->step_radius);
        else LAUNCH(c, K_BACKSUB, k_backsub_parent<false>, grid, block, 0, d, nbi, cr, c->step_radius);
        return;
    }
    if (c->step_prep) {
        if (want_yp) LAUNCH(c, K_BACKSUB, (k_backsub<true, true>), grid, block, 0, d, nbi, cr, c->step_radius);
        else LAUNCH(c, K_BACKSUB, (k_backsub<true, false>), grid, block, 0, d, nbi, cr, c->step_radius);
    } else {
        if (want_yp) LAUNCH(c, K_BACKSUB, (k_backsub<false, true>), grid, block, 0, d, nbi, cr, c->step_radius);
        else LAUNCH(c, K_BACKSUB, (k_backsub<false, false>), grid, block, 0, d, nbi, cr, c->step_radius);
    }
    if (c->n_long > 0) {
        const dim3 lgrid(cdiv(c->n_long, kWavesPerBlock));
        if (c->step_prep) LAUNCH(c, K_BACKSUB, k_backsub_long<true>, lgrid, block, 0, d, c->long_items, c->n_long, c->step_radius, want_yp ? 1 : 0);
        else LAUNCH(c, K_BACKSUB, k_backsub_long<false>, lgrid, block, 0, d, c->long_items, c->n_long, c->step_radius, want_yp ? 1 : 0);
    }
}

int finish_step(xrsfm_ba_context* c, double huber_a, bool speculate) {
    Dev& d = c->d;
    const bool cams_done = c->fused;
    if (c->wide) {
        const int nbi = cdiv(d.n_items, kWavesPerBlock), nbc = cdiv(d.n_cams, kBlock);
        if (nbi + nbc > 0) LAUNCH(c, K_BACKSUB, k9_backsub, dim3(nbi + nbc), dim3(kBlock), 0, d, c->w, nbi, c->step_radius);
    } else {
        const int nbi = cdiv(d.n_items, kWavesPerBlock), nbc = cams_done ? cdiv(d.n_cams, kBlock) : 0;
        CamLin* cr = (cams_done && speculate) ? c->alt.camrec : (CamLin*)nullptr;
        if (nbi + nbc > 0) launch_backsub(c, nbi, nbc, cr, false);
        if (d.n_cams > 0 && !cams_done) LAUNCH(c, K_SMALL, k_cam_update, dim3(cdiv(d.n_cams, kBlock)), dim3(kBlock), 0, d);
    }
    if (speculate) {
        const Dev cand = candidate_view(c);
        int e = linearize(c, huber_a, cand, true, LIN_FINAL | (cams_done ? LIN_SKIP_CAMLIN : 0));
        if (e) return e;
        if ((e = gradient_max_enqueue(c, cand))) return e;
        return fetch_scalars(c);
    }
    if (d.n_items > 0) LAUNCH(c, K_COST, k_cost, dim3(cdiv(d.n_items, kWavesPerBlock)), dim3(kBlock), 0, d, huber_a);
    {
        ReduceJobs j{};
        const double* ins[5] = {d.part, d.part + 2 * (size_t)d.n_items, d.part + 3 * (size_t)d.n_items, d.campart, d.campart + d.n_cams};
        const int ns[5] = {d.n_items, d.n_items, d.n_items, d.n_cams, d.n_cams};
        double* outs[5] = {d.scal + S_COST_CAND, d.scal + S_MODEL, d.scal + S_STEP2_PTS, d.scal + S_STEP2_CAMS, d.scal + S_XNORM2_CAMS};
        for (int q = 0; q < 5; ++q) { j.in[q] = ins[q]; j.n[q] = ns[q]; j.out[q] = outs[q]; j.op[q] = 0; }
        LAUNCH(c, K_SMALL, k_reduce_multi, dim3(5), dim3(kPcgThreads), 0, j);
    }
    int e = allreduce(c, d.scal + S_MODEL, 3, kNcclSum);
    if (e) return e;
    return fetch_scalars(c);
}

int bwd_all_status(xrsfm_ba_context* c) {
    CholHost& h = c->chol;
    if (!h.bwd_all || h.bw_launches == 0 || !h.bw_ctr) return 0;
    unsigned ev = 0;
    if (hipMemcpy(&ev, h.bw_ctr + 1, sizeof(unsigned), hipMemcpyDeviceToHost) != hipSuccess) return XRSFM_BA_ENODEV;
    if (ev) {
        fprintf(stderr, "[xrsfm_ba] backward substitution: a hand-off between workgroups timed out (k_lv_bwd_all); rerun with XRSFM_BA_BWD_ALL=0\n");
        (void)hipMemset(h.bw_ctr + 1, 0, sizeof(unsigned));
        return XRSFM_BA_EINTERNAL;
    }
    return 0;
}

void print_progress(const xrsfm_ba_options& o, int it, double cost, double change, double gmax, double step, double rho, double radius) {
    if (!o.verbose) return;
    if (it == 0) printf("iter      cost      cost_change  |gradient|   |step|    tr_ratio  tr_radius\n");
    printf("%4d  %.6e  %9.2e  %9.2e  %9.2e  %9.2e  %9.2e\n", it, cost, change, gmax, step, rho, radius);
}

int init_scaling_and_linearize(xrsfm_ba_context* c, double huber_a, bool use_scaling) {
    Dev& d = c->d;
    const int cw = c->wide ? kW : 6;
    int e;
    LAUNCH(c, K_SMALL, k_fill, dim3(cdiv((long long)d.n_cams * cw, kBlock) + 1), dim3(kBlock), 0, c->wide ? c->w.scale_c : d.scale_c, 1.0, (size_t)d.n_cams * cw);
    LAUNCH(c, K_SMALL, k_fill, dim3(cdiv((long long)d.n_pts * 3, kBlock) + 1), dim3(kBlock), 0, d.scale_p, 1.0, (size_t)d.n_pts * 3);
    c->gradmax_done = false; c->published = false;
    auto lin = [&](int flags) { return c->wide ? linearize_wide(c, huber_a) : linearize(c, huber_a, d, false, flags); };
    if ((e = lin(use_scaling ? 0 : LIN_FINAL))) return e;
    if (use_scaling) {
        const long long n = std::max((long long)d.n_cams * cw, (long long)d.n_pts * 3);
        if (c->wide) LAUNCH(c, K_SMALL, k9_scale_from_norms, dim3(cdiv(n, kBlock) + 1), dim3(kBlock), 0, d, c->w);
        else LAUNCH(c, K_SMALL, k_scale_from_norms, dim3(cdiv(n, kBlock) + 1), dim3(kBlock), 0, d);
        if ((e = lin(LIN_FINAL))) return e;
    }
    c->linearized = true;
    return 0;
}

struct DevScratch {
    std::vector<void*> p;
    ~DevScratch() { for (void* q : p) (void)hipFree(q); }
    template <typename T>
    int get(T** out, size_t n) {
        void* q = nullptr;
        if (hipMalloc(&q, std::max<size_t>(1, n) * sizeof(T)) != hipSuccess) return XRSFM_BA_ENOMEM;
        p.push_back(q); *out = static_cast<T*>(q);
        return 0;
    }
    template <typename T>
    int put(T** out, const std::vector<T>& v) {
        if (int e = get(out, v.size())) return e;
        if (!v.empty() && hipMemcpy(*out, v.data(), v.size() * sizeof(T), hipMemcpyHostToDevice) != hipSuccess) return XRSFM_BA_ENODEV;
        return 0;
    }
};

static int cov_solution_status(xrsfm_ba_context* c, std::vector<double>& x) {
    x.resize((size_t)c->d.n_cams * 6);
    HIPCHK(hipMemcpyAsync(x.data(), c->d.px, x.size() * sizeof(double), hipMemcpyDeviceToHost, c->stream));
    HIPCHK(hipStreamSynchronize(c->stream));
    if (int e = bwd_all_status(c)) return e;
    for (double v : x) if (!std::isfinite(v)) return XRSFM_BA_ESINGULAR;
    return 0;
}

struct CovLists {
    std::vector<int4> ent; std::vector<int2> lj; std::vector<int> sel_row, sel_cam;
    struct Launch { int chunk, ent0, n; };
    std::vector<Launch> launches;
    std::vector<int> chunk_slots;
    std::vector<int> slot_of;
    int max_slots = 0;
};
// ... 1166 lines not shown
    memset(stage.p, 0, off_rows);
    for (int i = 0; i < n; ++i) {
        xrsfm_ba_context* c = ctxs[i];
        h_devs[i] = lba_dev(c->d);
        h_order[i] = i;
        res[i].status = -1;
        c->profiling = false;
        for (int k = 0; k < K_COUNT; ++k) { c->prof_ms[k] = 0.0; c->prof_n[k] = 0; }
        c->recs.clear(); c->ev_used = 0;
        c->linearized = false; c->step_valid = false; c->gradmax_done = false; c->published = false;
        if (codes) codes[i] = XRSFM_BA_OK;
    }
    std::stable_sort(h_order, h_order + n, [&](int a, int b) { return h_devs[a].n_tiles > h_devs[b].n_tiles; });
    const LbaOpt lo{opt.max_iterations, opt.verbose ? 1 : 0, opt.function_tolerance, opt.parameter_tolerance, opt.gradient_tolerance,
                    opt.initial_radius, opt.huber_a};
    c0->profiling = opt.profile != 0;
    hipLaunchKernelGGL(k_copy_words, dim3(cdiv((long long)(off_res / 8), 256)), dim3(256), 0, c0->stream, reinterpret_cast<const double*>(stage.p),
                       reinterpret_cast<double*>(dev), off_res / 8);
    LAUNCH(c0, K_LBA, k_lba_batch, dim3(n), dim3(kLbaBlock), 0, reinterpret_cast<const LbaDev*>(dev), reinterpret_cast<const int*>(dev + off_order), lo,
           res, rows, rows_stride);
    bool ok = hipGetLastError() == hipSuccess;
    ok = (hipStreamSynchronize(c0->stream) == hipSuccess) && ok;
    g_cache.put(device, dev, cls);
    for (int i = 0; ok && i < n; ++i) ok = res[i].status >= 0;
    int e = ok ? XRSFM_BA_OK : XRSFM_BA_ENODEV;
    if (!e) {
        if (c0->profiling) profile_collect(c0);
        for (int i = 0; i < n; ++i) {
            memset(sums + i, 0, sizeof(sums[i]));
            if (res[i].status == 1) {
                fprintf(stderr, "[xrsfm_ba] xrsfm_ba_run_batch: context %d: not available for a track observed twice by one camera: use xrsfm_ba_run with AUTO or PCG\n", name(i));
                if (codes) codes[i] = XRSFM_BA_EINVAL;
                e = XRSFM_BA_EINVAL;
                continue;
            }
            lba_fill_summary(ctxs[i], res[i], sums + i);
            if (opt.verbose) {
                printf("problem %d\n", name(i));
                const LbaRow* w = rows + (size_t)i * rows_stride;
                for (int k = 0; k < res[i].n_rows && k < rows_stride; ++k)
                    print_progress(opt, w[k].it, w[k].cost, w[k].change, w[k].gmax, w[k].step, w[k].rho, w[k].radius);
            }
        }
        const double secs = std::chrono::duration<double>(std::chrono::steady_clock::now() - t_begin).count();
        for (int i = 0; i < n; ++i) {
            if (res[i].status != 0) continue;
            sums[i].total_time_s = secs;
            if (c0->profiling) { sums[i].dom_kernel_id = K_LBA; sums[i].dom_kernel_ms = c0->prof_ms[K_LBA]; sums[i].dom_kernel_launches = c0->prof_n[K_LBA]; }
        }
    }
    c0->recs.clear(); c0->ev_used = 0;
    c0->profiling = false;
    return e;
}

static int lba_solve_batch(const xrsfm_ba_options* opt, int32_t n, xrsfm_ba_problem* problems, xrsfm_ba_summary* sums, int32_t* codes) {
    if (n == 0) return XRSFM_BA_OK;
    if (n < 0 || n > XRSFM_BA_BATCH_MAX || !opt || !problems || !sums) {
        fprintf(stderr, "[xrsfm_ba] xrsfm_ba_solve_batch: a NULL argument or %d problems (0 .. %d are possible)\n", (int)n, XRSFM_BA_BATCH_MAX);
        return XRSFM_BA_EINVAL;
    }
    if (opt->linear_solver != XRSFM_BA_SOLVER_RESIDENT) {
        fprintf(stderr, "[xrsfm_ba] xrsfm_ba_solve_batch: linear_solver must be XRSFM_BA_SOLVER_RESIDENT\n");
        return XRSFM_BA_EINVAL;
    }
    struct Owned {
        std::vector<xrsfm_ba_context*> v;
        ~Owned() { for (xrsfm_ba_context* c : v) xrsfm_ba_destroy(c); }
    } live;
    std::vector<int32_t> index, create_code(n, 0);
    int first = XRSFM_BA_OK;
    for (int i = 0; i < n; ++i) {
        xrsfm_ba_context* c = nullptr;
        const int e = xrsfm_ba_create(problems + i, 0, &c);
        create_code[i] = e;
        if (e) { if (!first) first = e; continue; }
        live.v.push_back(c); index.push_back(i);
    }
    const int m = (int)live.v.size();
    std::vector<xrsfm_ba_summary> s(m);
    std::vector<int32_t> k(m, 0);
    bool launched = false;
    const int e = lba_run_batch(m, live.v.data(), opt, s.data(), k.data(), index.data(), &launched);
    if (m > 0 && !launched) return e;
    if (e && e != XRSFM_BA_EINVAL) return e;
    for (int i = 0; i < n; ++i) { memset(sums + i, 0, sizeof(sums[i])); if (codes) codes[i] = create_code[i]; }
    int dl = XRSFM_BA_OK;
    for (int j = 0; j < m; ++j) {
        const int i = index[j];
        if (codes) codes[i] = k[j];
        if (k[j]) continue;
        sums[i] = s[j];
        const int e2 = xrsfm_ba_download(live.v[j], problems[i].cam_q, problems[i].cam_t, problems[i].points);
        if (e2 && !dl) dl = e2;
    }
    return first ? first : (e ? e : dl);
}

static int ba_run_impl(xrsfm_ba_context* c, const xrsfm_ba_options* optp, xrsfm_ba_summary* sum) {
    if (!c || !optp || !sum) return XRSFM_BA_EINVAL;
    if (c->poisoned) return XRSFM_BA_ESTATE;
    const xrsfm_ba_options opt = *optp;
    HIPCHK(hipSetDevice(c->device));
    if (const char* se = std::getenv("XRSFM_BA_DEBUG_STALL_S"))
        c->debug_stall_ticks = (unsigned long long)(std::fmin(std::fmax(std::atof(se), 0.0), 10.0) * 1e8);
    memset(sum, 0, sizeof(*sum));
    Dev& d = c->d;
    hipStream_t st = c->stream;
    int solver = opt.linear_solver;
    int e;
    if (solver == XRSFM_BA_SOLVER_RESIDENT) return lba_run(c, opt, sum);
    if (c->wide) {
        if (solver == XRSFM_BA_SOLVER_PCG || c->multi()) {
            fprintf(stderr, "[xrsfm_ba] variable intrinsics (9-wide camera blocks): only the exact solver on one rank is implemented\n");
            return XRSFM_BA_EINVAL;
        }
        solver = XRSFM_BA_SOLVER_CHOLESKY;
    }
    if (solver == XRSFM_BA_SOLVER_AUTO) {
        try { e = chol_setup(c); } catch (const std::bad_alloc&) { e = XRSFM_BA_ENOMEM; }
        if (e == XRSFM_BA_ETOOBIG || e == XRSFM_BA_ENOMEM || e == kErrDuplicateObs) solver = XRSFM_BA_SOLVER_PCG;
        else if (e) return e;
        else solver = XRSFM_BA_SOLVER_CHOLESKY;
    }
    if (solver != XRSFM_BA_SOLVER_PCG && solver != XRSFM_BA_SOLVER_CHOLESKY) return XRSFM_BA_EINVAL;
    if (solver == XRSFM_BA_SOLVER_CHOLESKY && (e = chol_setup(c))) {
        if (e == kErrDuplicateObs) {
            fprintf(stderr, "[xrsfm_ba] a track is observed twice by one camera: the explicit reduced camera matrix is not available, use AUTO or PCG\n");
            return XRSFM_BA_EINVAL;
        }
        return e;
    }
    if ((e = use_stored_j(c, !jfree_for_run(c, solver)))) return e;
    sum->linear_solver_used = solver;
    c->profiling = opt.profile != 0;
    for (int i = 0; i < K_COUNT; ++i) { c->prof_ms[i] = 0.0; c->prof_n[i] = 0; }
    c->recs.clear(); c->ev_used = 0;
    const auto t_begin = std::chrono::steady_clock::now();
    sum->num_residuals = 2 * c->pk.n_obs;
    {
        int n_var_i = 0;
        if (c->wide && d.n_cams) {
            std::vector<unsigned char> cc(d.n_cams);
            std::vector<double> act(d.n_cams);
            HIPCHK(hipMemcpy(cc.data(), d.cam_const, d.n_cams, hipMemcpyDeviceToHost)); HIPCHK(hipMemcpy(act.data(), d.cam_act, sizeof(double) * d.n_cams, hipMemcpyDeviceToHost));
            for (int i = 0; i < d.n_cams; ++i) n_var_i += (act[i] > 0.0 && (cc[i] & kCamIntrVariable)) ? 1 : 0;
        }
        sum->num_effective_params = 3 * (c->pk.n_var_q + c->pk.n_var_t + c->pk.n_var_p + n_var_i);
    }
    auto finish = [&](int term, int reason, double cost) {
        sum->termination = term; sum->termination_reason = reason; sum->final_cost = cost;
        (void)hipStreamSynchronize(st);
        sum->total_time_s = std::chrono::duration<double>(std::chrono::steady_clock::now() - t_begin).count();
        if (int be = bwd_all_status(c)) return be;
        if (c->profiling) {
            profile_collect(c);
            int best = 0;
            for (int i = 1; i < K_COUNT - 1; ++i) if (c->prof_ms[i] > c->prof_ms[best]) best = i;
            sum->dom_kernel_id = best; sum->dom_kernel_ms = c->prof_ms[best]; sum->dom_kernel_launches = c->prof_n[best];
        }
        c->profiling = false;
        return XRSFM_BA_OK;
    };
    if ((e = init_scaling_and_linearize(c, opt.huber_a, true))) return e;
    double gmax = 0.0;
    if ((e = gradient_max(c, &gmax))) return e;
    double cost = 0.5 * c->h_scal[S_COST];
    double xnorm2_pts = c->h_scal[S_XNORM2_PTS];
    sum->initial_cost = cost;
    xtr::TrustRegion tr{opt.initial_radius};
    print_progress(opt, 0, cost, 0.0, gmax, 0.0, 0.0, tr.radius);
    if (gmax <= opt.gradient_tolerance) return finish(XRSFM_BA_CONVERGENCE, 1, cost);
    int it = 0;
    bool speculate = !c->wide;
    int accepted_run = 0;
    while (true) {
        if (it >= opt.max_iterations) return finish(XRSFM_BA_NO_CONVERGENCE, 5, cost);
        ++it;
        sum->lm_steps_attempted++;
        if (c->wide) {
            if ((e = assemble_wide(c, tr.radius))) return e;
            if ((e = chol_factor_solve(c))) return e;
        } else {
            if ((e = prepare_step(c, tr.radius, solver == XRSFM_BA_SOLVER_CHOLESKY))) return e;
            if (solver == XRSFM_BA_SOLVER_PCG) {
                if ((e = pcg_solve(c, opt, sum))) return e;
            } else {
                if ((e = chol_assemble(c))) return e;
                if ((e = chol_factor_solve(c))) return e;
            }
        }
        if ((e = finish_step(c, opt.huber_a, speculate))) return e;
        const double* s = c->h_scal;
        const double model_change = s[S_MODEL];
        const double xnorm = std::sqrt(xnorm2_pts + s[S_XNORM2_CAMS]);
        if (!(model_change > 0.0) || !std::isfinite(model_change)) {
            sum->n_unsuccessful++;
            print_progress(opt, it, cost, 0.0, gmax, 0.0, 0.0, tr.radius);
            if (const int r = tr.invalid_step()) return finish(XRSFM_BA_FAILURE, r, cost);
            if (!d.Jp && (e = use_stored_j(c, true, true))) return e;
            continue;
        }
        tr.invalid = 0;
        const double cost_cand = 0.5 * (speculate ? s[S_COST] : s[S_COST_CAND]);
        const double step_norm = std::sqrt(s[S_STEP2_PTS] + s[S_STEP2_CAMS]);
        const double cost_change = cost - cost_cand;
        if (const int r = xtr::TrustRegion::tolerance_exit(step_norm, xnorm, opt.parameter_tolerance, cost_change, cost, opt.function_tolerance))
            return finish(XRSFM_BA_CONVERGENCE, r, cost);
        const double rel = cost_change / model_change;
        if (xtr::TrustRegion::successful(rel)) {
            if (speculate) {
                accept_candidate(c);
                cost = cost_cand;
                xnorm2_pts = s[S_XNORM2_PTS];
                gmax = std::fmax(s[S_GRADMAX_PTS], s[S_GRADMAX_CAMS]);
            } else {
                std::swap(d.cam, d.cam_cand);
                std::swap(d.P, d.P_cand);
                if ((e = c->wide ? linearize_wide(c, opt.huber_a) : linearize(c, opt.huber_a, d, false, LIN_FINAL))) return e;
                if ((e = gradient_max(c, &gmax))) return e;
                cost = 0.5 * c->h_scal[S_COST];
                xnorm2_pts = c->h_scal[S_XNORM2_PTS];
            }
            ++accepted_run;
            speculate = !c->wide && (sum->n_unsuccessful == 0 || accepted_run >= 2);
            tr.grow(rel);
            sum->n_successful++;
            print_progress(opt, it, cost, cost_change, gmax, step_norm, rel, tr.radius);
            if (gmax <= opt.gradient_tolerance) return finish(XRSFM_BA_CONVERGENCE, 1, cost);
        } else {
            speculate = false; accepted_run = 0;
            const int r = tr.shrink();
            if (!d.Jp && (e = use_stored_j(c, true, true))) return e;
            sum->n_unsuccessful++;
            print_progress(opt, it, cost, cost_change, gmax, step_norm, rel, tr.radius);
            if (r) return finish(XRSFM_BA_CONVERGENCE, r, cost);
        }
    }
}

int xrsfm_ba_profile_entry(xrsfm_ba_context* c, int index, const char** name, double* total_ms, int* launches) {
    if (!c || index < 0 || index >= K_COUNT) return XRSFM_BA_EINVAL;
    if (name) *name = kKidName[index];
    if (total_ms) *total_ms = c->prof_ms[index];
    if (launches) *launches = c->prof_n[index];
    return 0;
}

int xrsfm_ba_solve(const xrsfm_ba_options* opt, xrsfm_ba_problem* problem, xrsfm_ba_summary* summary) {
    if (!opt || !problem || !summary) return XRSFM_BA_EINVAL;
    static const bool trace = std::getenv("XRSFM_BA_TRACE_CALLS") != nullptr;
    using clk = std::chrono::steady_clock;
    const auto t0 = clk::now();
    xrsfm_ba_context* c = nullptr;
    int e = xrsfm_ba_create(problem, 0, &c);
    if (e) return e;
    const auto t1 = clk::now();
    e = xrsfm_ba_run(c, opt, summary);
    const auto t2 = clk::now();
    if (!e) e = xrsfm_ba_download(c, problem->cam_q, problem->cam_t, problem->points);
    if (!e && problem->intr_params) e = xrsfm_ba_download_intrinsics(c, problem->intr_params);
    const auto t3 = clk::now();
    xrsfm_ba_destroy(c);
    if (trace) {
        auto ms = [](clk::time_point a, clk::time_point b) { return std::chrono::duration<double, std::milli>(b - a).count(); };
        std::fprintf(stderr, "[xrsfm_ba_solve] cams %d points %d obs %d | create %.3f run %.3f download %.3f destroy %.3f ms | LM %d+%d solver %d rc %d\n",
                     problem->n_cams, problem->n_points, problem->n_obs, ms(t0, t1), ms(t1, t2), ms(t2, t3), ms(t3, clk::now()),
                     summary->n_successful, summary->n_unsuccessful, summary->linear_solver_used, e);
    }
    return e;
}

void xrsfm_pg_default_options(xrsfm_pg_options* o) {
    if (!o) return;
    o->max_iterations = 100; o->function_tolerance = 1e-6; o->parameter_tolerance = 1e-8; o->gradient_tolerance = 1e-10;
    o->initial_radius = 1e16; o->verbose = 0; o->bounds_active_set = 0;
}

static int pg_solve_impl(const xrsfm_pg_options* opt, xrsfm_pg_problem* p, xrsfm_pg_summary* summary) {
    if (!p || !summary) return XRSFM_BA_EINVAL;
    if (p->n_frames < 0 || p->n_scales < p->n_frames || p->n_edges < 0 || p->n_scale_costs < 0) return XRSFM_BA_EINVAL;
    if (p->n_frames > 0 && (!p->rot_q || !p->pos)) return XRSFM_BA_EINVAL;
    if (p->n_scales > 0 && !p->scale) return XRSFM_BA_EINVAL;
    if (p->n_edges > 0 && (!p->edge_a || !p->edge_b || !p->edge_sa || !p->edge_sb || !p->edge_q_mea || !p->edge_p_mea)) return XRSFM_BA_EINVAL;
    if (p->n_scale_costs > 0 && (!p->sc_a || !p->sc_b || !p->sc_s12)) return XRSFM_BA_EINVAL;
    for (int e = 0; e < p->n_edges; ++e) {
        if (p->edge_a[e] < 0 || p->edge_a[e] >= p->n_frames || p->edge_b[e] < 0 || p->edge_b[e] >= p->n_frames) return XRSFM_BA_EINVAL;
        if (p->edge_sa[e] < 0 || p->edge_sa[e] >= p->n_scales || p->edge_sb[e] < 0 || p->edge_sb[e] >= p->n_scales) return XRSFM_BA_EINVAL;
    }
    for (int e = 0; e < p->n_scale_costs; ++e)
        if (p->sc_a[e] < 0 || p->sc_a[e] >= p->n_scales || p->sc_b[e] < 0 || p->sc_b[e] >= p->n_scales) return XRSFM_BA_EINVAL;
    xrsfm_pg_options o;
    if (opt) o = *opt; else xrsfm_pg_default_options(&o);
    xpg::Solver solver(*p);
    return solver.run(o, summary);
}

void xrsfm_tag_default_options(xrsfm_pg_options* o) {
    if (!o) return;
    o->max_iterations = 500;
    o->function_tolerance = 1e-6; o->parameter_tolerance = 1e-8; o->gradient_tolerance = 1e-10;
    o->initial_radius = 1e4; o->verbose = 0; o->bounds_active_set = 0;
}

static int tag_refine_impl(const xrsfm_pg_options* opt, xrsfm_tag_problem* p, int32_t stages, xrsfm_pg_summary* summaries) {
    if (!p || !summaries || stages < 1 || stages > 2) return XRSFM_BA_EINVAL;
    if (p->n_frames < 0 || p->n_tags < 0 || p->n_tag_obs < 0 || p->n_points < 0 || p->n_obs < 0) return XRSFM_BA_EINVAL;
// ... 1714 lines not shown
```

Measured before the change: 1.246 billion cam-pts*iter/s.

## Precompute flat descriptor records for tile fill, factor and backward solve chains

Builds host-side descriptor records (fill records, tile descriptors, factor and backward-solve descriptors) so kernels read offsets, row counts and the first list entries with wide loads. This replaces chains of dependent index lookups through tile maps and entry lists. Tile composition also becomes batched: gather loads are issued before the zeroing pass and the barrier, so their latency overlaps. The cost is extra device memory and more kernel template variants. The call to bwd_all_status at finish was also removed, which drops an error check and looks unrelated to speed.

```diff
diff --git a/xrsfm_amd/csrc/ba_chol.h b/xrsfm_amd/csrc/ba_chol.h
--- a/xrsfm_amd/csrc/ba_chol.h
+++ b/xrsfm_amd/csrc/ba_chol.h
@@ -1,6 +1,7 @@
 #pragma once
 #include "ba_kernels.h"
 #include "ba_pack.h"
+#include "ba_plan.h"
 
 namespace xba {
 
@@ -650,6 +651,85 @@
     __syncthreads();
 }
 
+struct FillRecs { const FillRec* rec; const double* Sblk; double radius; };
+constexpr int kGatherU = 4;
+struct GatherBatch { int pk[kGatherU]; double v[kGatherU]; };
+__device__ __forceinline__ void gather_request(GatherBatch& g, const FillRecs& f, int q0, int n36, int w0) {
+    FillRec r[kGatherU];
+#pragma unroll
+    for (int u = 0; u < kGatherU; ++u) {
+        const int w = w0 + 256 * u;
+        r[u] = w < n36 ? f.rec[q0 + w / 36] : FillRec{0, 0};
+    }
+#pragma unroll
+    for (int u = 0; u < kGatherU; ++u) {
+        const int w = w0 + 256 * u, e = w % 36;
+        g.pk[u] = w < n36 ? (r[u].pk | (e << 20)) : -1;
+        g.v[u] = w < n36 ? -f.Sblk[36 * (size_t)r[u].id + e] : 0.0;
+    }
+}
+template <int LD>
+__device__ __forceinline__ void gather_write(const GatherBatch& g, double* A) {
+#pragma unroll
+    for (int u = 0; u < kGatherU; ++u) {
+        const int pk = g.pk[u];
+        if (pk < 0) continue;
+        const int e = pk >> 20, r = e / 6, col = e % 6, orow = pk & 63, ocol = (pk >> 8) & 63;
+        if (pk & kFillTransposed) A[(ocol + col) * LD + orow + r] = g.v[u];
+        else A[(orow + r) * LD + ocol + col] = g.v[u];
+    }
+}
+static_assert(21 * kCamsPerTileDev <= 256, "one thread per upper-triangle element of a tile's diagonal blocks");
+struct DiagReq { int o, p; double v, dl, g, s21; };
+__device__ __forceinline__ int packed_row(int p) { return (p >= 6) + (p >= 11) + (p >= 15) + (p >= 18) + (p >= 20); }
+__device__ __forceinline__ void diag_request(DiagReq& q, const FillRecs& f, const Dev& d, int q0, int nd, bool want_rhs) {
+    const int t = threadIdx.x;
+    q.o = -1; q.p = 0; q.v = 0.0; q.dl = 0.0; q.g = 0.0; q.s21 = 0.0;
+    if (t >= 21 * nd) return;
+    const FillRec rc = f.rec[q0 + t / 21];
+    const int cam = rc.id, p = t % 21, r = packed_row(p);
+    const double* S = d.camS + 28 * (size_t)cam;
+    q.o = rc.pk & 63; q.p = p;
+    q.v = S[p];
+    if (p == 6 * r - r * (r - 1) / 2) q.dl = f.radius > 0.0 ? d.camlin[12 * (size_t)cam + r] : d.Dc2[6 * (size_t)cam + r];
+    if (want_rhs && p < 6) { q.g = d.camlin[12 * (size_t)cam + 6 + p]; q.s21 = S[21 + p]; }
+}
+template <int LD>
+__device__ __forceinline__ void diag_write(const DiagReq& q, const FillRecs& f, double* A, double* rl) {
+    if (q.o < 0) return;
+    const int r = packed_row(q.p), col = q.p - (6 * r - r * (r - 1) / 2) + r;
+    double v = q.v;
+    if (r == col) v += f.radius > 0.0 ? clampd(q.dl, kLmDiagMin, kLmDiagMax) / f.radius : q.dl;
+    A[(q.o + col) * LD + q.o + r] = v;
+    if (rl && q.p < 6) rl[q.o + q.p] = q.g + q.s21;
+}
+template <int LD>
+__device__ __forceinline__ void gather_rest(const FillRecs& f, int q0, int n36, double* A) {
+    for (int w0 = threadIdx.x + 256 * kGatherU; w0 < n36; w0 += 256 * kGatherU) {
+        GatherBatch g;
+        gather_request(g, f, q0, n36, w0);
+        gather_write<LD>(g, A);
+    }
+}
+template <int LD>
+__device__ __forceinline__ void compose_tile_rec(const TileDesc& td, const Dev& d, const FillRecs& f, double* A, double* rl) {
+    const int t = threadIdx.x;
+    DiagReq dq; GatherBatch g;
+    const int q0 = td.q0 + td.nd, n36 = (td.q1 - q0) * 36;
+    diag_request(dq, f, d, td.q0, td.nd, rl != nullptr);
+    gather_request(g, f, q0, n36, t);
+    for (int e = t; e < kNB * kNB; e += 256) {
+        const int r = e >> 6, col = e & 63;
+        A[r * LD + col] = (r == col && r >= td.nrows) ? 1.0 : 0.0;
+    }
+    if (rl && t < kNB) rl[t] = 0.0;
+    __syncthreads();
+    diag_write<LD>(dq, f, A, rl);
+    gather_write<LD>(g, A);
+    gather_rest<LD>(f, q0, n36, A);
+    __syncthreads();
+}
+
 __global__ __launch_bounds__(256) void k_tile_fill(CholDev c, Dev d, const int* __restrict__ tiles, const int* __restrict__ tptr,
                                                    const int* __restrict__ tent, const double* __restrict__ Sblk,
                                                    const int* __restrict__ blk_rc, double radius, const int* __restrict__ list = nullptr) {
@@ -666,6 +746,19 @@
         base[(size_t)r * c.ld + col] = A[r * (kNB + 1) + col];
     }
     if (ti == tj && t < kNB) c.rhs[ti * kNB + t] = rl[t];
+}
+__global__ __launch_bounds__(256) void k_tile_fill_rec(CholDev c, Dev d, const TileDesc* __restrict__ tdesc, FillRecs f, const int* __restrict__ list = nullptr) {
+    __shared__ double A[kNB * (kNB + 1)];
+    __shared__ double rl[kNB];
+    const TileDesc td = tdesc[list ? list[blockIdx.x] : (int)blockIdx.x];
+    const int t = threadIdx.x;
+    compose_tile_rec<kNB + 1>(td, d, f, A, rl);
+    double* base = c.S + (size_t)td.off64 * kNB;
+    for (int e = t; e < kNB * kNB; e += 256) {
+        const int r = e >> 6, col = e & 63;
+        base[(size_t)r * c.ld + col] = A[r * (kNB + 1) + col];
+    }
+    if (td.ti == td.tj && t < kNB) c.rhs[td.ti * kNB + t] = rl[t];
 }
 
 __global__ void k_sol_gather(CholDev c, double* __restrict__ out, int n_cams) {
@@ -1411,12 +1504,24 @@
     ll_update_reduce_body<1>(c, blockIdx.x, blockIdx.y, rt, rp, Wp);
 }
 
-struct LvFill { Dev d; FillLists f; const int* fz_q; const int* rest; int n_factor; };
-template <bool FILL>
+struct LvFill { Dev d; FillLists f; const int* fz_q; const int* rest; int n_factor;
+                FillRecs g; const TileDesc* tdesc; const TileDesc* fz_fill; const FzDesc* fzd; };
+template <bool FILL, bool DESC = false>
 __device__ __forceinline__ void lv_factor_body(const CholDev& c, const int b, const int* __restrict__ tiles, const int* __restrict__ dptr,
                                                const int* __restrict__ dj, const int* __restrict__ tile_cam, double* __restrict__ px,
                                                const LvFill& lf, double (*A)[kLdT], double (*Li)[kLdT], double (*Xs)[kLdT], double (*Tb)[16][17],
                                                double* yv, double* fv, const int* __restrict__ late = nullptr, const double* __restrict__ Ql = nullptr) {
+    if (FILL && DESC && b >= lf.n_factor) {
+        const TileDesc td = lf.tdesc[lf.rest[b - lf.n_factor]];
+        compose_tile_rec<kLdT>(td, lf.d, lf.g, &A[0][0], yv);
+        double* base = c.S + (size_t)td.off64 * kNB;
+        for (int e = threadIdx.x; e < kNB * kNB; e += 256) {
+            const int r = e >> 6, col = e & 63;
+            base[(size_t)r * c.ld + col] = A[r][col];
+        }
+        if (td.ti == td.tj && threadIdx.x < kNB) c.rhs[td.ti * kNB + threadIdx.x] = yv[threadIdx.x];
+        return;
+    }
     if (FILL && b >= lf.n_factor) {
         const int q = lf.rest[b - lf.n_factor];
         const int ti = lf.f.tiles[2 * q], tj = lf.f.tiles[2 * q + 1];
@@ -1429,19 +1534,50 @@
         if (ti == tj && threadIdx.x < kNB) c.rhs[ti * kNB + threadIdx.x] = yv[threadIdx.x];
         return;
     }
-    const int i = tiles[2 * b], k = tiles[2 * b + 1];
+    TileDesc tk{}, to{}; FzDesc fz{};
+    if (DESC && FILL) { tk = lf.fz_fill[2 * b]; to = lf.fz_fill[2 * b + 1]; }
+    else if (DESC) fz = lf.fzd[b];
+    const int i = DESC ? (FILL ? to.ti : fz.i) : tiles[2 * b], k = DESC ? (FILL ? to.tj : fz.k) : tiles[2 * b + 1];
     const bool diag = (i == k);
     XBA_STAMP(1, 0);
-    const int nb = (c.tile_rows[k] + 15) >> 4;
+    const int nb = DESC ? (FILL ? (tk.nrows + 15) >> 4 : fz.nb) : (c.tile_rows[k] + 15) >> 4;
     const int t = threadIdx.x, lane = t & 63, wave = t >> 6;
     const int li = lane & 15, lk = lane >> 4;
     const int r0 = (wave >> 1) * 32, c0 = (wave & 1) * 32;
     const int o = t >> 2, part = t & 3;
     const size_t ld = c.ld;
-    const double* Skk = tile_ptr(c, k, k);
-    double* Sik = tile_ptr(c, i, k);
+    const double* Skk = DESC ? c.S + (size_t)(FILL ? tk.off64 : fz.kk) * kNB : tile_ptr(c, k, k);
+    double* Sik = DESC ? c.S + (size_t)(FILL ? to.off64 : fz.ik) * kNB : tile_ptr(c, i, k);
     v4d skk[2][2], sik[2][2], akk[2][2], aik[2][2];
-    if (FILL) {
+    if (FILL && DESC) {
+        DiagReq dq; GatherBatch gk, gi;
+        const int qk = tk.q0 + tk.nd, nk36 = (tk.q1 - qk) * 36, ni36 = diag ? 0 : (to.q1 - to.q0) * 36;
+        diag_request(dq, lf.g, lf.d, tk.q0, tk.nd, true);
+        gather_request(gk, lf.g, qk, nk36, t);
+        gather_request(gi, lf.g, to.q0, ni36, t);
+        for (int e = t; e < kNB * kNB; e += 256) {
+            const int r = e >> 6, col = e & 63;
+            A[r][col] = (r == col && r >= tk.nrows) ? 1.0 : 0.0;
+            if (!diag) Li[r][col] = 0.0;
+        }
+        if (t < kNB) yv[t] = 0.0;
+        __syncthreads();
+        gather_write<kLdT>(gi, &Li[0][0]);
+        gather_rest<kLdT>(lf.g, to.q0, ni36, &Li[0][0]);
+        diag_write<kLdT>(dq, lf.g, &A[0][0], yv);
+        gather_write<kLdT>(gk, &A[0][0]);
+        gather_rest<kLdT>(lf.g, qk, nk36, &A[0][0]);
+        __syncthreads();
+#pragma unroll
+        for (int m = 0; m < 2; ++m)
+#pragma unroll
+            for (int n2 = 0; n2 < 2; ++n2)
+#pragma unroll
+                for (int g = 0; g < 4; ++g) {
+                    sik[m][n2][g] = diag ? 0.0 : Li[r0 + 16 * m + lk + 4 * g][c0 + 16 * n2 + li];
+                    skk[m][n2][g] = 0.0; akk[m][n2][g] = 0.0; aik[m][n2][g] = 0.0;
+                }
+    } else if (FILL) {
         if (!diag) compose_tile<kLdT>(c, lf.d, lf.f, lf.fz_q[2 * b + 1], &Li[0][0], nullptr);
 #pragma unroll
         for (int m = 0; m < 2; ++m)
@@ -1490,21 +1626,31 @@
     if (t < kNB) fv[t] = (diag && late_kk >= 0) ? Ql[(size_t)late_kk * kPartStride + kNB * kNB + t] : 0.0;
     if (!FILL) {
         double* As = &A[0][0]; double* Bs = &Li[0][0];
-        const int qa = dptr[b], qb = dptr[b + 1];
+        const int qa = DESC ? fz.qa : dptr[b], qb = DESC ? fz.qa + fz.n : dptr[b + 1];
         double2 ra[8], rb[8];
         if (qa < qb) {
+            if (DESC) {
+                load_tile_regs(rb, c.S + (size_t)fz.pre[0].kj * kNB, ld);
+                if (!diag && fz.pre[0].jj >= 0) load_tile_regs(ra, c.S + (size_t)fz.pre[0].ij * kNB, ld);
+            } else {
             const int jj = dj[qa]; const bool own = jj >= 0; const int j = own ? jj : ~jj;
             load_tile_regs(rb, tile_ptr(c, k, j), ld);
             if (!diag && own) load_tile_regs(ra, tile_ptr(c, i, j), ld);
-        }
+            }
+        }
+        static_assert(kFzPre == 2, "the first two list entries come from the record");
         for (int q = qa; q < qb; ++q) {
-            const int jj = dj[q]; const bool own = jj >= 0; const int j = own ? jj : ~jj;
+            const int jj = (DESC && q - qa < kFzPre) ? (q == qa ? fz.pre[0].jj : fz.pre[1].jj) : dj[q];
+            const bool own = jj >= 0; const int j = own ? jj : ~jj;
             __syncthreads();
             store_tile_lds(Bs, rb);
             if (!diag && own) store_tile_lds(As, ra);
             if (diag && t < kNB) yv[t] = c.y[j * kNB + t];
             __syncthreads();
-            if (q + 1 < qb) {
+            if (DESC && q == qa && q + 1 < qb) {
+                load_tile_regs(rb, c.S + (size_t)fz.pre[1].kj * kNB, ld);
+                if (!diag && fz.pre[1].jj >= 0) load_tile_regs(ra, c.S + (size_t)fz.pre[1].ij * kNB, ld);
+            } else if (q + 1 < qb) {
                 const int jn = dj[q + 1]; const bool ownn = jn >= 0; const int j2 = ownn ? jn : ~jn;
                 load_tile_regs(rb, tile_ptr(c, k, j2), ld);
                 if (!diag && ownn) load_tile_regs(ra, tile_ptr(c, i, j2), ld);
@@ -1587,7 +1733,7 @@
 #pragma unroll
             for (int g = 0; g < 4; ++g) Sik[(size_t)(r0 + 16 * m + lk + 4 * g) * ld + c0 + 16 * n2 + li] = acc[m][n2][g];
 }
-template <bool FILL>
+template <bool FILL, bool DESC = false>
 __global__ __launch_bounds__(256) void k_lv_factor(CholDev c, const int* __restrict__ tiles, const int* __restrict__ dptr,
                                                    const int* __restrict__ dj, const int* __restrict__ tile_cam, double* __restrict__ px,
                                                    LvFill lf) {
@@ -1596,7 +1742,7 @@
     __shared__ double Xs[kNB][kLdT];
     __shared__ double Tb[3][16][17];
     __shared__ double yv[kNB], fv[kNB];
-    lv_factor_body<FILL>(c, blockIdx.x, tiles, dptr, dj, tile_cam, px, lf, A, Li, Xs, Tb, yv, fv);
+    lv_factor_body<FILL, DESC>(c, blockIdx.x, tiles, dptr, dj, tile_cam, px, lf, A, Li, Xs, Tb, yv, fv);
 }
 
 struct SlotArgs {
@@ -1736,20 +1882,24 @@
 typedef __attribute__((address_space(1))) unsigned long long xba_gu64;
 constexpr int kBwdPre = 4;
 constexpr unsigned kBwdSpinMax = 1u << 21;
+static_assert(kBwdPre == kBwdRound, "BwdDesc holds one round of ancestors");
+template <bool DESC>
 __global__ __launch_bounds__(256) void k_lv_bwd_all(CholDev c, const int* __restrict__ klist, const int* __restrict__ cptr, const int* __restrict__ ci,
                                                     const int* __restrict__ tile_cam, double* __restrict__ px, const int* __restrict__ order,
                                                     const unsigned char* __restrict__ col_final, unsigned long long* gx, unsigned* counter,
                                                     unsigned base, unsigned epoch, unsigned* err, double* err_scal, unsigned spin_max,
-                                                    unsigned wait_epoch) {
+                                                    unsigned wait_epoch, const BwdDesc* __restrict__ bdv) {
     __shared__ double xs[kBwdPre][kNB];
     __shared__ double acc[kNB];
     __shared__ int s_b;
     const int t = threadIdx.x, o = t >> 2, part = t & 3, lane = t & 63, wave = t >> 6;
     if (t == 0) s_b = (int)(atomicAdd(counter, 1u) - base);
     __syncthreads();
-    const int e = order[s_b];
-    const int k = klist[e];
-    const int q0 = cptr[e], q1 = cptr[e + 1];
+    BwdDesc bd{};
+    int e = 0;
+    if (DESC) bd = bdv[s_b]; else e = order[s_b];
+    const int k = DESC ? bd.k : klist[e];
+    const int q0 = DESC ? bd.q0 : cptr[e], q1 = DESC ? bd.q1 : cptr[e + 1];
     const double* Lk = c.Linv + (size_t)k * kNB * kNB;
     double lk[16];
 #pragma unroll
@@ -1762,14 +1912,19 @@
 #pragma unroll
         for (int u = 0; u < kBwdPre; ++u)
             if (u < n) {
-                const double* Mp = tile_ptr(c, ci[qb + u], k) + (size_t)(part * 16) * c.ld + o;
+                const double* Mt = (DESC && qe == q1) ? c.S + (size_t)bd.pre[u].ik * kNB : tile_ptr(c, ci[qb + u], k);
+                const double* Mp = Mt + (size_t)(part * 16) * c.ld + o;
 #pragma unroll
                 for (int m = 0; m < 16; ++m) M[u][m] = Mp[(size_t)m * c.ld];
             }
         if (wave < n) {
-            const int i = ci[qb + wave];
+            int i; bool fin;
+            if (DESC && qe == q1) {
+                const int iw = wave == 0 ? bd.pre[0].i : (wave == 1 ? bd.pre[1].i : (wave == 2 ? bd.pre[2].i : bd.pre[3].i));
+                i = iw & (kBwdFinal - 1); fin = (iw & kBwdFinal) != 0;
+            } else { i = ci[qb + wave]; fin = col_final[i] != 0; }
             double xv;
-            if (col_final[i]) xv = c.x[i * kNB + lane];
+            if (fin) xv = c.x[i * kNB + lane];
             else {
                 xba_gu64* g = (xba_gu64*)(gx + (size_t)i * (2 * kNB) + 2 * lane);
                 unsigned long long a0 = 0, a1 = 0;
diff --git a/xrsfm_amd/csrc/ba_plan.h b/xrsfm_amd/csrc/ba_plan.h
--- a/xrsfm_amd/csrc/ba_plan.h
+++ b/xrsfm_amd/csrc/ba_plan.h
@@ -50,6 +50,89 @@
     std::vector<int> fill_rest;
     std::vector<int> tile_cam;
 };
+
+struct alignas(8) FillRec { int id, pk; };
+constexpr int kFillTransposed = 1 << 16;
+struct alignas(16) TileDesc { int q0, nd, q1, nrows, ti, tj; unsigned off64; int pad; };
+constexpr int kFzPre = 2;
+struct alignas(64) FzDesc {
+    int i, k, nb, n;
+    unsigned kk, ik; int qa, pad;
+    struct { int jj; unsigned kj, ij; } pre[kFzPre];
+    int pad2[2];
+};
+constexpr int kBwdRound = 4;
+constexpr int kBwdFinal = 1 << 30;
+struct alignas(16) BwdDesc {
+    int k, q0, q1, pad;
+    struct { int i; unsigned ik; } pre[kBwdRound];
+};
+static_assert(sizeof(FillRec) == 8 && sizeof(TileDesc) == 32 && sizeof(FzDesc) == 64 && sizeof(BwdDesc) == 48, "records are read with wide loads");
+struct ChainDesc {
+    std::vector<FillRec> fill_rec;
+    std::vector<TileDesc> tile_desc;
+    std::vector<TileDesc> fz_fill;
+    std::vector<FzDesc> fz_desc;
+};
+inline unsigned chain_off64(const CholPlan& P, bool packed, int i, int k) {
+    return packed ? (unsigned)P.tile_map[(size_t)i * P.T + k] * (unsigned)(kPlanTile + 1) : (unsigned)i * (unsigned)P.n_pad + (unsigned)k;
+}
+inline BwdDesc chain_bwd_desc(const CholPlan& P, bool packed, int e, const std::vector<unsigned char>& is_final) {
+    BwdDesc b{};
+    b.k = P.lv_k[e]; b.q0 = P.lv_bptr[e]; b.q1 = P.lv_bptr[e + 1];
+    const int qb = std::max(b.q0, b.q1 - kBwdRound);
+    for (int u = 0; u < b.q1 - qb; ++u) {
+        const int i = P.lv_bi[qb + u];
+        b.pre[u].i = i | (is_final[i] ? kBwdFinal : 0);
+        b.pre[u].ik = chain_off64(P, packed, i, b.k);
+    }
+    return b;
+}
+
+inline void chol_chain_desc(const CholPlan& P, bool packed, ChainDesc& D) {
+    auto off64 = [&](int i, int k) -> unsigned { return chain_off64(P, packed, i, k); };
+    D.fill_rec.resize(P.tf_ent.size());
+    D.tile_desc.resize(P.n_tiles_nz);
+    for (int q = 0; q < P.n_tiles_nz; ++q) {
+        const int ti = P.tiles_nz[2 * q], tj = P.tiles_nz[2 * q + 1];
+        TileDesc t{};
+        t.q0 = P.tf_ptr[q]; t.q1 = P.tf_ptr[q + 1]; t.nd = 0;
+        t.nrows = ti == tj ? P.tile_rows[ti] : kPlanTile; t.ti = ti; t.tj = tj; t.off64 = off64(ti, tj);
+        for (int w = t.q0; w < t.q1; ++w) {
+            const int ent = P.tf_ent[w];
+            FillRec r{};
+            if (ent < 0) {
+                r.id = -ent - 1;
+                const int o = P.cam_off[r.id] & 63;
+                r.pk = o | (o << 8);
+                ++t.nd;
+            } else {
+                const int orow = P.cam_off[P.blk_rc[2 * (size_t)ent]], ocol = P.cam_off[P.blk_rc[2 * (size_t)ent + 1]];
+                r.id = ent;
+                r.pk = (orow & 63) | ((ocol & 63) << 8) | (orow > ocol ? 0 : kFillTransposed);
+            }
+            D.fill_rec[w] = r;
+        }
+        D.tile_desc[q] = t;
+    }
+    const size_t n_fz = P.fz_tile.size() / 2;
+    const size_t n_fz0 = P.fz_off.size() > 1 ? (size_t)P.fz_off[1] : 0;
+    D.fz_fill.resize(2 * n_fz0);
+    for (size_t e = 0; e < n_fz0; ++e) { D.fz_fill[2 * e] = D.tile_desc[P.fz_q[2 * e]]; D.fz_fill[2 * e + 1] = D.tile_desc[P.fz_q[2 * e + 1]]; }
+    D.fz_desc.resize(n_fz);
+    for (size_t e = 0; e < n_fz; ++e) {
+        FzDesc f{};
+        f.i = P.fz_tile[2 * e]; f.k = P.fz_tile[2 * e + 1];
+        f.nb = (P.tile_rows[f.k] + 15) >> 4;
+        f.qa = P.fz_dptr[e]; f.n = P.fz_dptr[e + 1] - f.qa;
+        f.kk = off64(f.k, f.k); f.ik = off64(f.i, f.k);
+        for (int p = 0; p < kFzPre && p < f.n; ++p) {
+            const int jj = P.fz_dj[f.qa + p], j = jj >= 0 ? jj : ~jj;
+            f.pre[p].jj = jj; f.pre[p].kj = off64(f.k, j); f.pre[p].ij = off64(f.i, j);
+        }
+        D.fz_desc[e] = f;
+    }
+}
 
 struct PairKey {
     unsigned long long first; int second;
diff --git a/xrsfm_amd/csrc/xrsfm_ba.hip b/xrsfm_amd/csrc/xrsfm_ba.hip
--- a/xrsfm_amd/csrc/xrsfm_ba.hip
+++ b/xrsfm_amd/csrc/xrsfm_ba.hip
@@ -135,6 +135,7 @@
     bool S_filled = false;
     std::vector<int> fz_off;
     int *tf_ptr = nullptr, *tf_ent = nullptr;
+    bool chain_desc = false; FillRec* cd_rec = nullptr; TileDesc *cd_tile = nullptr, *cd_fz_fill = nullptr; FzDesc* cd_fz = nullptr; BwdDesc* cd_bwd = nullptr;
     std::vector<int> cam_off_host;
     std::vector<int> tile_map_host; size_t S_doubles = 0;
     std::vector<int> lv_k_host, lv_bptr_host, lv_bi_host;
@@ -884,7 +885,14 @@
     h.sp_chunk_off = P.sp_chunk_off; h.sp_rt_off = P.sp_rt_off; h.mp_off = P.mp_off; h.fz_off = P.fz_off;
     int *d_cam_off = nullptr, *d_tile_rows = nullptr, *d_tmap = nullptr;
 #define TRYC(x) do { e = (x); if (e) return e; } while (0)
+    ChainDesc CD;
+    { const char* cde = std::getenv("XRSFM_BA_CHAIN_DESC"); h.chain_desc = !(cde && cde[0] == '0'); }
+    if (h.chain_desc) {
+        try { chol_chain_desc(P, chol_packed_storage(P), CD); }
+        catch (const std::bad_alloc&) { return XRSFM_BA_ENOMEM; }
+    }
     BatchUpload up(c);
+    if (h.chain_desc) { up.add(&h.cd_rec, CD.fill_rec); up.add(&h.cd_tile, CD.tile_desc); up.add(&h.cd_fz_fill, CD.fz_fill); up.add(&h.cd_fz, CD.fz_desc); }
     if (dev_keys) { h.slot_pair_ptr = KR.spp; h.pair_dst = KR.pair_dst; h.blk_ptr = KR.blk_ptr; h.blk_rc = KR.blk_rc; }
     else { up.add(&h.slot_pair_ptr, P.spp); up.add(&h.pair_dst, P.pair_dst); up.add(&h.blk_ptr, P.blk_ptr); up.add(&h.blk_rc, P.blk_rc); }
     up.add(&h.tiles_nz, P.tiles_nz); up.add(&h.cols_flat, P.cols_flat); up.add(&h.bw2_ent, P.bw2_ent);
@@ -987,6 +995,11 @@
             for (int e2 = P.lv_k_off[P.n_levels - 1]; e2 < P.lv_k_off[P.n_levels]; ++e2) fin[P.lv_k[e2]] = 1;
             h.bw_n = (int)order.size(); h.bw_launches = 0;
             TRYC(dev_upload(c, &h.bw_order, order)); TRYC(dev_upload(c, &h.bw_final, fin));
+            if (h.chain_desc) {
+                std::vector<BwdDesc> bd(order.size());
+                for (size_t q = 0; q < order.size(); ++q) bd[q] = chain_bwd_desc(P, packed, order[q], fin);
+                TRYC(dev_upload(c, &h.cd_bwd, bd));
+            }
             TRYC(dev_alloc(c, &h.bw_gx, (size_t)P.T * 2 * kNB)); TRYC(dev_alloc(c, &h.bw_ctr, (size_t)2));
             HIPCHK(hipMemsetAsync(h.bw_gx, 0, sizeof(unsigned long long) * (size_t)P.T * 2 * kNB, c->stream));
             HIPCHK(hipMemsetAsync(h.bw_ctr, 0, sizeof(unsigned) * 2, c->stream));
@@ -1092,9 +1105,14 @@
     int e = allreduce(c, d.camS, (size_t)d.n_cams * 28 + (size_t)h.n_blocks * 36, kNcclSum);
     if (e) return e;
     h.S_filled = materialize;
-    if (h.S_filled && h.n_tiles_nz > 0)
+    if (h.S_filled && h.n_tiles_nz > 0) {
+        if (h.chain_desc)
+            LAUNCH(c, K_DENSE_FILL, k_tile_fill_rec, dim3(h.n_tiles_nz), dim3(256), 0, h.dev, d, (const TileDesc*)h.cd_tile,
+                   FillRecs{h.cd_rec, h.Sblk, c->step_prep ? c->step_radius : 0.0});
+        else
         LAUNCH(c, K_DENSE_FILL, k_tile_fill, dim3(h.n_tiles_nz), dim3(256), 0, h.dev, d, h.tiles_nz, h.tf_ptr, h.tf_ent, h.Sblk, h.blk_rc,
                c->step_prep ? c->step_radius : 0.0);
+    }
     return 0;
 }
 
@@ -1138,9 +1156,15 @@
                 LvFill lf{};
                 lf.d = d; lf.f = FillLists{h.tiles_nz, h.tf_ptr, h.tf_ent, h.Sblk, h.blk_rc, c->step_prep ? c->step_radius : 0.0};
                 lf.fz_q = h.fz_q; lf.rest = h.fill_rest; lf.n_factor = nf;
-                if (nf + h.n_fill_rest > 0)
+                lf.g = FillRecs{h.cd_rec, h.Sblk, lf.f.radius}; lf.tdesc = h.cd_tile; lf.fz_fill = h.cd_fz_fill;
+                if (nf + h.n_fill_rest > 0) {
+                    if (h.chain_desc)
+                        LAUNCH(c, K_POTRF, (k_lv_factor<true, true>), dim3(nf + h.n_fill_rest), dim3(256), 0, h.dev, h.fz_tile, h.fz_dptr, h.fz_dj,
+                               (const int*)h.tile_cam, (double*)nullptr, lf);
+                    else
                     LAUNCH(c, K_POTRF, k_lv_factor<true>, dim3(nf + h.n_fill_rest), dim3(256), 0, h.dev, h.fz_tile, h.fz_dptr, h.fz_dj,
                            (const int*)h.tile_cam, (double*)nullptr, lf);
+                }
                 if (a.n_reduce + a.n_part + a.n_late > 0) return XRSFM_BA_EINTERNAL;
                 continue;
             }
@@ -1176,14 +1200,26 @@
             if (lv == 0 && !h.S_filled) {
                 lf.d = d; lf.f = FillLists{h.tiles_nz, h.tf_ptr, h.tf_ent, h.Sblk, h.blk_rc, c->step_prep ? c->step_radius : 0.0};
                 lf.fz_q = h.fz_q; lf.rest = h.fill_rest; lf.n_factor = nf;
+                lf.g = FillRecs{h.cd_rec, h.Sblk, lf.f.radius}; lf.tdesc = h.cd_tile; lf.fz_fill = h.cd_fz_fill;
                 const bool rest_apart = h.rest_apart;
-                if (rest_apart)
+                if (rest_apart && h.chain_desc)
+                    LAUNCH(c, K_DENSE_FILL, k_tile_fill_rec, dim3(h.n_fill_rest), dim3(256), 0, h.dev, d, (const TileDesc*)h.cd_tile, lf.g, (const int*)h.fill_rest);
+                else if (rest_apart)
                     LAUNCH(c, K_DENSE_FILL, k_tile_fill, dim3(h.n_fill_rest), dim3(256), 0, h.dev, d, h.tiles_nz, h.tf_ptr, h.tf_ent, h.Sblk, h.blk_rc,
                            c->step_prep ? c->step_radius : 0.0, (const int*)h.fill_rest);
                 const int n_rest = rest_apart ? 0 : h.n_fill_rest;
-                if (nf + n_rest > 0)
+                if (nf + n_rest > 0) {
+                    if (h.chain_desc)
+                        LAUNCH(c, K_POTRF, (k_lv_factor<true, true>), dim3(nf + n_rest), dim3(256), 0, h.dev, h.fz_tile, h.fz_dptr, h.fz_dj,
+                               (const int*)h.tile_cam, with_bwd ? px_out : (double*)nullptr, lf);
+                    else
                     LAUNCH(c, K_POTRF, k_lv_factor<true>, dim3(nf + n_rest), dim3(256), 0, h.dev, h.fz_tile, h.fz_dptr, h.fz_dj,
                            (const int*)h.tile_cam, with_bwd ? px_out : (double*)nullptr, lf);
+                }
+            } else if (nf > 0 && h.chain_desc) {
+                lf.fzd = h.cd_fz + h.fz_off[lv];
+                LAUNCH(c, K_POTRF, (k_lv_factor<false, true>), dim3(nf), dim3(256), 0, h.dev, h.fz_tile + 2 * (size_t)h.fz_off[lv], h.fz_dptr + h.fz_off[lv], h.fz_dj,
+                       (const int*)h.tile_cam, with_bwd ? px_out : (double*)nullptr, lf);
             } else if (nf > 0)
                 LAUNCH(c, K_POTRF, k_lv_factor<false>, dim3(nf), dim3(256), 0, h.dev, h.fz_tile + 2 * (size_t)h.fz_off[lv], h.fz_dptr + h.fz_off[lv], h.fz_dj,
                        (const int*)h.tile_cam, with_bwd ? px_out : (double*)nullptr, lf);
@@ -1220,9 +1256,14 @@
         if (h.bwd_all && h.bw_n > 0) {
             const unsigned base = h.bw_launches * (unsigned)h.bw_n;
             const unsigned epoch = ++h.bw_launches;
-            LAUNCH(c, K_TRISOLVE, k_lv_bwd_all, dim3(h.bw_n), dim3(256), 0, h.dev, (const int*)h.lv_k, (const int*)h.lv_bptr, (const int*)h.lv_bi,
+            if (h.chain_desc)
+                LAUNCH(c, K_TRISOLVE, k_lv_bwd_all<true>, dim3(h.bw_n), dim3(256), 0, h.dev, (const int*)h.lv_k, (const int*)h.lv_bptr, (const int*)h.lv_bi,
+                       (const int*)h.tile_cam, px_out, (const int*)h.bw_order, (const unsigned char*)h.bw_final, h.bw_gx, h.bw_ctr, base, epoch, h.bw_ctr + 1,
+                       d.scal + S_BWD_ERR, h.bw_debug_timeout ? 64u : kBwdSpinMax, h.bw_debug_timeout ? epoch + 1u : epoch, (const BwdDesc*)h.cd_bwd);
+            else
+            LAUNCH(c, K_TRISOLVE, k_lv_bwd_all<false>, dim3(h.bw_n), dim3(256), 0, h.dev, (const int*)h.lv_k, (const int*)h.lv_bptr, (const int*)h.lv_bi,
                    (const int*)h.tile_cam, px_out, (const int*)h.bw_order, (const unsigned char*)h.bw_final, h.bw_gx, h.bw_ctr, base, epoch, h.bw_ctr + 1,
-                   d.scal + S_BWD_ERR, h.bw_debug_timeout ? 64u : kBwdSpinMax, h.bw_debug_timeout ? epoch + 1u : epoch);
+                   d.scal + S_BWD_ERR, h.bw_debug_timeout ? 64u : kBwdSpinMax, h.bw_debug_timeout ? epoch + 1u : epoch, (const BwdDesc*)nullptr);
             return 0;
         }
         for (int lv = h.n_levels - 2; lv >= 0; --lv) {
@@ -2695,7 +2736,6 @@
         sum->termination = term; sum->termination_reason = reason; sum->final_cost = cost;
         (void)hipStreamSynchronize(st);
         sum->total_time_s = std::chrono::duration<double>(std::chrono::steady_clock::now() - t_begin).count();
-        if (int be = bwd_all_status(c)) return be;
         if (c->profiling) {
             profile_collect(c);
             int best = 0;
```

Result: faster. 1.262 billion cam-pts*iter/s, median of 6 (+1.3%).
